# HaoZhongkai/DPOT

Measured on AMD Instinct MI355X. Metric: PDE samples/sec (128^2 x10 -> 1 rollout step), DPOT-Tiny train step, higher is better.
Workload: dtype f32

## Files before the change

dpot_amd/_lib.py:

```python
from __future__ import annotations

import ctypes as C
import os
import threading

HERE = os.path.dirname(os.path.abspath(__file__))
LIB_PATH = os.environ.get("DPOT_HIP_LIB") or os.path.join(HERE, "lib", "libdpot_hip.so")

c_fp = C.c_void_p
c_i = C.c_int
c_i64 = C.c_int64
c_f = C.c_float
c_d = C.c_double


class GemmDesc(C.Structure):
    _fields_ = [
        ("A", c_fp), ("B", c_fp), ("C", c_fp),
        ("M", C.c_int32), ("N", C.c_int32), ("K", C.c_int32),
        ("batch", C.c_int32),
        ("transA", C.c_int32), ("transB", C.c_int32),
        ("lda", C.c_int32), ("ldb", C.c_int32), ("ldc", C.c_int32),
        ("strideA", c_i64), ("strideB", c_i64), ("strideC", c_i64),
        ("bias", c_fp), ("strideBias", c_i64),
        ("act", C.c_int32), ("epi_mode", C.c_int32),
        ("aux", c_fp), ("ldaux", C.c_int32), ("strideAux", c_i64),
        ("preact", c_fp), ("ldpre", C.c_int32), ("stridePre", c_i64),
        ("res", c_fp), ("ldres", C.c_int32), ("res_div", C.c_int32), ("res_mod", C.c_int32),
        ("strideRes", c_i64),
        ("accumulate", C.c_int32), ("splitk", C.c_int32),
        ("workspace", c_fp),
        ("tile", C.c_int32),
        ("tag", C.c_int32),
        ("colsum_out", c_fp), ("strideColsum", c_i64), ("colsum_of", C.c_int32),
        ("precision", C.c_int32),
    ]


class PackJob(C.Structure):
    _fields_ = [("src", c_fp), ("dst", c_fp), ("rows", C.c_int32), ("K", C.c_int32), ("ld", C.c_int32),
                ("trans", C.c_int32)]


class AdamPackJob(C.Structure):
    _fields_ = [("off", C.c_int64), ("dst_rows", c_fp), ("dst_trans", c_fp), ("R", C.c_int32), ("K", C.c_int32),
                ("tile0", C.c_int32), ("pad_", C.c_int32)]


class AdamRange(C.Structure):
    _fields_ = [("start", C.c_int64), ("len", C.c_int64)]


class LambChunk(C.Structure):
    _fields_ = [("off", C.c_int64), ("len", C.c_int32), ("tensor", C.c_int32)]


class LambTensor(C.Structure):
    _fields_ = [("first_chunk", C.c_int32), ("n_chunks", C.c_int32)]


class LayoutJob(C.Structure):
    _fields_ = [("src", c_fp), ("add", c_fp), ("dst", c_fp), ("d0", C.c_int32), ("d1", C.c_int32), ("d2", C.c_int32),
                ("v0", C.c_int32), ("v1", C.c_int32), ("v2", C.c_int32), ("s0", C.c_int64), ("s1", C.c_int64),
                ("s2", C.c_int64)]


class AfnoPackJob(C.Structure):
    _fields_ = [("w", c_fp), ("b", c_fp), ("wbig", c_fp), ("bbig", c_fp), ("fwd", c_fp), ("bwd", c_fp)]


class SampleDesc(C.Structure):
    _fields_ = [("data", c_fp), ("H", C.c_int32), ("W", C.c_int32), ("T", C.c_int32), ("C", C.c_int32),
                ("t0", C.c_int32), ("reserved", C.c_int32)]


SIGNATURES = {
    "dpot_version": (c_i, []),
    "dpot_tune": (c_i, [C.c_char_p, c_i]),
    "dpot_last_error": (C.c_char_p, []),
    "dpot_gemm_f32": (c_i, [C.POINTER(GemmDesc), c_fp]),
    "dpot_gemm_workspace_bytes": (c_i64, [C.POINTER(GemmDesc)]),
    "dpot_gemm_auto_splitk": (c_i, [c_i, c_i, c_i, c_i]),
    "dpot_gemm_auto_splitk2": (c_i, [c_i, c_i, c_i, c_i, c_i]),
    "dpot_rfft2": (c_i, [c_fp, c_fp] + [c_i] * 8 + [c_fp]),
    "dpot_rfft2_norm_supported": (c_i, [c_i, c_i, c_i]),
    "dpot_rfft2_norm": (c_i, [c_fp] * 5 + [c_i, c_fp] + [c_i] * 8 + [c_fp]),
    "dpot_irfft2_norm": (c_i, [c_fp] * 6 + [c_i, c_fp] + [c_i] * 8 + [c_fp]),
    "dpot_irfft2": (c_i, [c_fp, c_fp, c_fp] + [c_i] * 8 + [c_fp]),
    "dpot_afno_pack": (c_i, [c_fp] * 4 + [c_i, c_i, c_fp]),
    "dpot_afno_pack_multi": (c_i, [C.POINTER(C.c_void_p)] * 4 + [c_i, c_i, c_i, c_fp]),
    "dpot_afno_unpack_grad": (c_i, [c_fp] * 4 + [c_i, c_i, c_fp]),
    "dpot_afno_mlp2_supported": (c_i, [c_i, c_i]),
    "dpot_afno_mlp2": (c_i, [c_fp] * 9 + [c_i] * 8 + [c_fp]),
    "dpot_afno_mlp3_supported": (c_i, [c_i, c_i]),
    "dpot_afno_mlp6_supported": (c_i, [c_i, c_i]),
    "dpot_afno_pack6_elems": (c_i64, [c_i, c_i]),
    "dpot_afno_pack6": (c_i, [c_fp] * 3 + [c_i] * 3 + [c_fp]),
    "dpot_afno_mlp6": (c_i, [c_fp] * 9 + [c_i] * 7 + [c_fp]),
    "dpot_afno_block_weights": (c_i, [c_fp] * 3 + [c_i, c_i, c_fp]),
    "dpot_afno_pack_all": (c_i, [c_fp, c_i, c_i, c_i, c_i, c_fp]),
    "dpot_groupnorm_ws_elems": (c_i64, [c_i] * 4),
    "dpot_groupnorm_fwd": (c_i, [c_fp] * 7 + [c_i] * 4 + [c_f, c_fp]),
    "dpot_groupnorm_bwd": (c_i, [c_fp] * 11 + [c_i] * 4 + [c_fp]),
    "dpot_groupnorm_bwd_packs_supported": (c_i, [c_i] * 3),
    "dpot_groupnorm_bwd_packs_rows": (c_i, [c_i] * 4),
    "dpot_groupnorm_bwd_packs": (c_i, [c_fp] * 12 + [c_i] * 4 + [c_fp]),
    "dpot_groupnorm_param_grads": (c_i, [C.c_void_p] * 3 + [c_i] * 3 + [c_fp]),
    "dpot_afno_fused_supported": (c_i, [c_i] * 7),
    "dpot_afno_fused_fwd": (c_i, [c_fp] * 19 + [c_i] * 9 + [c_f, c_fp]),
    "dpot_gn_dft_supported": (c_i, [c_i] * 4),
    "dpot_gn_rfft2": (c_i, [c_fp] * 6 + [c_i] * 8 + [c_f, c_fp]),
    "dpot_irfft2_gn": (c_i, [c_fp] * 12 + [c_i] * 9 + [c_f, c_fp]),
    "dpot_gn_bwd_rfft2": (c_i, [c_fp] * 8 + [c_i] * 9 + [c_fp]),
    "dpot_irfft2_gn_bwd": (c_i, [c_fp] * 9 + [c_i] * 9 + [c_fp]),
    "dpot_patchify": (c_i, [c_fp] * 5 + [c_i] * 6 + [c_fp]),
    "dpot_unpatchify": (c_i, [c_fp] * 2 + [c_i] * 6 + [c_fp]),
    "dpot_pixel_shuffle": (c_i, [c_fp] * 2 + [c_i] * 6 + [c_fp]),
    "dpot_copy2d_pad": (c_i, [c_fp, c_i, c_i, c_fp, c_i, c_i, c_fp]),
    "dpot_transpose2d": (c_i, [c_fp, c_fp, c_i, c_i, c_i, c_fp]),
    "dpot_colsum_parts": (c_i, [c_i]),
    "dpot_colsum": (c_i, [c_fp, c_i, c_i, c_i, c_fp, c_fp, c_fp]),
    "dpot_colsum_scatter": (c_i, [c_fp, c_i, c_i, c_i, c_fp, c_i, C.POINTER(C.c_int), C.POINTER(C.c_int),
                                  C.POINTER(C.c_void_p), c_fp]),
    "dpot_group_rowsum": (c_i, [c_fp, c_fp] + [c_i] * 4 + [c_fp]),
    "dpot_small_linear_supported": (c_i, [c_i] * 3),
    "dpot_small_linear": (c_i, [c_fp, c_i, c_fp, c_i, c_fp, c_fp, c_fp] + [c_i] * 5 + [c_fp]),
    "dpot_token_mean": (c_i, [c_fp, c_fp] + [c_i] * 3 + [c_fp]),
    "dpot_token_mean_bwd": (c_i, [c_fp] * 3 + [c_i] * 3 + [c_fp]),
    "dpot_bias_add": (c_i, [c_fp] * 3 + [c_i, c_i, c_fp]),
    "dpot_scale_shift": (c_i, [c_fp] * 4 + [c_i] * 3 + [c_fp]),
    "dpot_scale_shift_bwd": (c_i, [c_fp] * 6 + [c_i] * 3 + [c_fp]),
    "dpot_timeagg_scale_w": (c_i, [c_fp] * 4 + [c_i, c_i, c_fp]),
    "dpot_timeagg_scale_w_bwd": (c_i, [c_fp] * 6 + [c_i, c_i, c_fp]),
    "dpot_out_tail_partial_rows": (c_i, [c_i] * 4),
    "dpot_out_tail_partial_cols": (c_i, []),
    "dpot_out_tail_fwd": (c_i, [c_fp] * 6 + [c_i] * 6 + [c_fp]),
    "dpot_out_tail_bwd": (c_i, [c_fp] * 7 + [c_i] * 6 + [c_fp]),
    "dpot_rel_l2_chunks": (c_i, [c_i, c_i]),
    "dpot_rel_l2_fwd": (c_i, [c_fp] * 5 + [c_i] * 4 + [c_fp]),
    "dpot_rel_l2_bwd": (c_i, [c_fp] * 6 + [c_i] * 4 + [c_fp]),
    "dpot_sumsq": (c_i, [c_fp, c_i64, c_fp, c_fp, c_i, c_fp]),
    "dpot_adam_step": (c_i, [c_fp] * 4 + [c_i64, c_fp, c_fp, c_f, c_fp]),
    "dpot_adam_stage": (c_i, [c_fp, c_fp, c_f, c_d, c_d, c_f, c_f, c_f, c_i, c_fp]),
    "dpot_lamb_chunk_elems": (c_i, []),
    "dpot_lamb_step": (c_i, [c_fp] * 5 + [c_fp, c_f, c_fp, c_i, c_fp, c_i, c_fp, c_fp, c_i, c_fp]),
    "dpot_lamb_stage": (c_i, [c_fp, c_fp, c_d, c_d, c_d, c_f, c_f, c_f, c_f, c_i, c_i, c_fp]),
    "dpot_cls_ce_fwd": (c_i, [c_fp] * 4 + [c_i, c_i, c_fp]),
    "dpot_cls_ce_bwd": (c_i, [c_fp] * 5 + [c_i, c_i, c_fp]),
    "dpot_rel_l2_combine": (c_i, [c_fp, c_fp, c_i64, c_i, c_i, c_i, c_fp, c_fp]),
    "dpot_metrics_accum": (c_i, [c_fp] * 4 + [c_i, c_fp, c_f, c_i64, c_i64, c_i64, c_fp]),
    "dpot_noise_chunks": (c_i, [c_i, c_i]),
    "dpot_noise_inject": (c_i, [c_fp] * 4 + [c_f] + [c_i] * 3 + [c_fp]),
    "dpot_noise_inject_rng": (c_i, [c_fp] * 4 + [c_f] + [c_i] * 3 + [c_fp]),
    "dpot_noise_inject_bwd": (c_i, [c_fp] * 7 + [c_f] + [c_i] * 3 + [c_fp]),
    "dpot_window_slide": (c_i, [c_fp] * 3 + [c_i64] + [c_i] * 3 + [c_fp]),
    "dpot_window_slide_bwd": (c_i, [c_fp] * 3 + [c_i64] + [c_i] * 3 + [c_fp]),
    "dpot_resize_pad_window": (c_i, [c_fp, c_i, c_fp, c_fp] + [c_i] * 6 + [c_fp]),
    "dpot_spectral_resize_pad": (c_i, [c_i, c_i]),
    "dpot_spectral_resize": (c_i, [c_fp] * 7 + [c_i] * 6 + [c_fp]),
    "dpot_eval_metrics_pad": (c_i, [c_i, c_i]),
    "dpot_eval_metrics_max_size": (c_i, [c_i]),
    "dpot_eval_metrics_acc_elems": (c_i64, [c_i] * 4),
    "dpot_eval_metrics_stats": (c_i, [c_fp] * 9 + [c_i] * 4 + [c_fp]),
    "dpot_eval_metrics_finalize": (c_i, [c_fp] * 3 + [c_i] * 5 + [c_fp]),
    "dpot_panel_pack_weights": (c_i, [c_fp, c_i, c_i, c_fp]),
    "dpot_layout_jobs": (c_i, [c_fp, c_i, c_i64, c_fp]),
    "dpot_bf16_packed_elems": (c_i64, [c_i, c_i, c_i]),
    "dpot_bf16_pack_rows": (c_i, [c_fp, c_i, c_i, c_i, c_i, c_i, c_fp, c_fp]),
    "dpot_bf16_pack_jobs": (c_i, [c_fp, c_i, c_i, c_i, c_fp]),
    "dpot_adam_pack_supported": (c_i, [c_i, c_i]),
    "dpot_adam_step_packs": (c_i, [c_fp] * 6 + [c_f, c_fp, c_fp, c_i, c_fp, c_i, c_i, c_fp]),
    "dpot_gemm_bf16p_supported": (c_i, [c_i, c_i, c_i]),
    "dpot_gemm_bf16p": (c_i, [c_fp, c_fp, c_fp, c_fp, c_i, c_fp, c_i, c_fp, c_i, c_fp, c_i] + [c_i] * 7 + [c_fp] * 7),
    "dpot_gemm_bf16p_splitk": (c_i, [c_i, c_i, c_i]),
    "dpot_gemm_bf16p_pair_wanted": (c_i, [c_i] * 5),
    "dpot_gemm_bf16p_pair_splitk": (c_i, [c_i] * 5),
    "dpot_gemm_bf16p_kernel_kind": (c_i, [c_i] * 6),
    "dpot_gemm_bf16p_pair": (c_i, [c_fp, c_fp, c_fp, c_i, c_i, c_i, c_fp, c_fp, c_fp, c_i, c_i, c_i, c_i, c_i, c_fp, c_fp]),
    "dpot_gemm_tn_splitk": (c_i, [c_i] * 4),
    "dpot_mlp_wgrad2_splitk": (c_i, [c_i] * 3),
    "dpot_mlp_wgrad2_ws_elems": (c_i64, [c_i] * 3),
    "dpot_mlp_wgrad2": (c_i, [c_fp] * 4 + [c_i] * 3 + [c_fp] * 5 + [c_i, c_fp]),
    "dpot_afno_wgrad2_splitk": (c_i, [c_i] * 3),
    "dpot_afno_wgrad2_ws_elems": (c_i64, [c_i] * 3),
    "dpot_afno_wgrad2": (c_i, [c_fp] * 4 + [c_i] * 4 + [c_fp] * 5 + [c_i, c_fp]),
    "dpot_block_finalize": (c_i, [c_fp, c_i, c_i, c_i] + [c_fp] * 4 + [c_fp, c_i, c_i, c_i] + [c_fp] * 4 + [c_fp] * 3
                            + [c_i, c_i, c_i] + [c_fp] * 4 + [c_i, c_fp]),
    "dpot_bf16_pack_both_supported": (c_i, [c_i, c_i]),
    "dpot_bf16_pack_both": (c_i, [c_fp, c_i, c_i, c_i, c_fp, c_fp, c_fp, c_fp]),
    "dpot_bf16_pack_both_norm": (c_i, [c_fp, c_i, c_i, c_i, c_fp, c_fp, c_fp, c_fp, c_i, c_i, c_fp, c_fp, c_fp]),
    "dpot_embed_supported": (c_i, [c_i] * 5),
    "dpot_embed_wfrag_elems": (c_i, []),
    "dpot_embed_pack_w0": (c_i, [c_fp, c_i, c_fp, c_fp]),
    "dpot_embed_fwd": (c_i, [c_fp] * 5 + [c_i] * 6 + [c_fp]),
    "dpot_embed_wgrad_ws_elems": (c_i, [c_i] * 3),
    "dpot_embed_wgrad": (c_i, [c_fp] * 4 + [c_i] * 7 + [c_fp]),
    "dpot_gemm_panel_supported": (c_i, [c_i, c_i, c_i]),
    "dpot_gemm_panel": (c_i, [c_fp, c_i, c_fp, c_fp, c_fp, c_i, c_fp, c_i, c_fp, c_i, c_fp, c_i] + [c_i] * 5 + [c_fp]),
}

_lib = None
_lock = threading.Lock()


class DpotHipError(RuntimeError):
    pass


def lib_path() -> str:
    return LIB_PATH


def load():
    global _lib
    if _lib is not None:
        return _lib
    with _lock:
        if _lib is not None:
            return _lib
        if not os.path.exists(LIB_PATH):
            raise DpotHipError(
                f"{LIB_PATH} is missing - build it first (python -m dpot_amd.build, or __graft_entry__.build()). "
                "dpot_amd has no CPU / eager fallback by design.")
        lib = C.CDLL(LIB_PATH)
        for name, (res, args) in SIGNATURES.items():
            fn = getattr(lib, name)
            fn.restype = res
            fn.argtypes = args
        _lib = lib
    return _lib


def check(rc: int, what: str = "") -> None:
    if rc != 0:
# ... 3 lines not shown
```

dpot_amd/build.py:

```python
from __future__ import annotations

import os
import shutil
import subprocess
import sys
from concurrent.futures import ThreadPoolExecutor

HERE = os.path.dirname(os.path.abspath(__file__))
CSRC = os.path.join(HERE, "csrc")
LIBDIR = os.path.join(HERE, "lib")
LIB = os.path.join(LIBDIR, "libdpot_hip.so")
SOURCES = ["core.hip", "gemm.hip", "gemm_panel.hip", "gemm_tn.hip", "gemm_bf16p.hip", "afno_mlp.hip", "afno_mlp6.hip", "afno_fused.hip", "dft.hip", "norm.hip", "gn_dft.hip", "misc.hip", "loss_opt.hip", "metrics.hip", "tail.hip", "data.hip", "embed.hip", "resize.hip", "evalmetrics.hip"]
FLAGS = ["--offload-arch=gfx950", "-O3", "-std=c++17", "-fPIC", "-Wall", "-Wno-unused-function",
         "-Wno-pass-failed"]
EXTRA_FLAGS = {"afno_mlp6.hip": ["-fno-slp-vectorize"]}


def _hipcc() -> str:
    for cand in (os.environ.get("HIPCC"), shutil.which("hipcc"), "/opt/rocm/bin/hipcc"):
        if cand and os.path.exists(cand):
            return cand
    raise RuntimeError("hipcc not found (need ROCm >= 7.0 to build the gfx950 kernels)")


def _stale(target: str, deps) -> bool:
    if not os.path.exists(target):
        return True
    t = os.path.getmtime(target)
    return any(os.path.getmtime(d) > t for d in deps)


def build(force: bool = False, verbose: bool = True) -> str:
    hipcc = _hipcc()
    os.makedirs(LIBDIR, exist_ok=True)
    hdrs = [os.path.join(CSRC, "common.h"), os.path.join(CSRC, "dft_fast.h"), os.path.join(CSRC, "gemm_split.h"), os.path.join(CSRC, "gemm_epi.h"), os.path.join(CSRC, "gemm_bf16p_common.h"), os.path.join(os.path.dirname(HERE), "include", "dpot_hip.h")]
    objs, jobs = [], []
    for src in SOURCES:
        s = os.path.join(CSRC, src)
        o = os.path.join(LIBDIR, src.replace(".hip", ".o"))
        objs.append(o)
        if force or _stale(o, [s] + hdrs):
            jobs.append([hipcc] + FLAGS + EXTRA_FLAGS.get(src, []) + ["-c", s, "-o", o])

    def run(cmd):
        if verbose:
            print("[dpot_amd.build]", " ".join(cmd), flush=True)
        r = subprocess.run(cmd, capture_output=True, text=True)
        if r.returncode != 0:
            raise RuntimeError(f"hipcc failed:\n{' '.join(cmd)}\n{r.stdout}\n{r.stderr}")
        return r

    if jobs:
        with ThreadPoolExecutor(max_workers=min(6, len(jobs))) as ex:
            list(ex.map(run, jobs))
    if jobs or force or _stale(LIB, objs):
        run([hipcc, "--offload-arch=gfx950", "-shared", "-fPIC", "-o", LIB] + objs)
    return LIB


if __name__ == "__main__":
    print(build(force="--force" in sys.argv))
```

dpot_amd/csrc/gemm.hip:

```cpp
#include "common.h"
#include "gemm_epi.h"

namespace dpot {

constexpr int BK = 32;
constexpr int KPAD = 4;

template <int R, bool VEC>
__device__ __forceinline__ void load_kcontig(float4 (&reg)[R / 32], const float* __restrict__ base, int ld,
                                             int r0, int rmax, int k0, int kmax, int tid) {
#pragma unroll
  for (int i = 0; i < R / 32; ++i) {
    const int f = tid + 256 * i;
    const int r = r0 + (f >> 3);
    const int k = k0 + ((f & 7) << 2);
    const float* row = base + (long long)min(r, rmax - 1) * ld;
    float4 v;
    if constexpr (VEC) {
      v = *reinterpret_cast<const float4*>(row + min(k, kmax - 4));
    } else {
      const int kl = kmax - 1;
      v.x = row[min(k + 0, kl)]; v.y = row[min(k + 1, kl)]; v.z = row[min(k + 2, kl)]; v.w = row[min(k + 3, kl)];
    }
    reg[i] = v;
  }
}
template <int R, bool VEC>
__device__ __forceinline__ void load_rcontig(float4 (&reg)[R / 32], const float* __restrict__ base, int ld,
                                             int r0, int rmax, int k0, int kmax, int tid) {
  constexpr int F4_PER_ROW = R / 4;
#pragma unroll
  for (int i = 0; i < R / 32; ++i) {
    const int f = tid + 256 * i;
    const int k = k0 + f / F4_PER_ROW;
    const int r = r0 + ((f % F4_PER_ROW) << 2);
    const float* row = base + (long long)min(k, kmax - 1) * ld;
    float4 v;
    if constexpr (VEC) {
      v = *reinterpret_cast<const float4*>(row + min(r, rmax - 4));
    } else {
      const int rl = rmax - 1;
      v.x = row[min(r + 0, rl)]; v.y = row[min(r + 1, rl)]; v.z = row[min(r + 2, rl)]; v.w = row[min(r + 3, rl)];
    }
    reg[i] = v;
  }
}
template <int R>
__device__ __forceinline__ void zero_tail_kcontig(float* lds, int krem, int tid) {
  for (int idx = tid; idx < R * BK; idx += 256) {
    const int r = idx / BK, k = idx % BK;
    if (k >= krem) lds[r * (BK + KPAD) + k] = 0.f;
  }
}
template <int R>
__device__ __forceinline__ void zero_tail_rcontig(float* lds, int krem, int tid) {
  for (int idx = tid + krem * R; idx < BK * R; idx += 256) lds[idx] = 0.f;
}
template <int R>
__device__ __forceinline__ void store_kcontig(float* lds, const float4 (&reg)[R / 32], int tid) {
#pragma unroll
  for (int i = 0; i < R / 32; ++i) {
    const int f = tid + 256 * i;
    *reinterpret_cast<float4*>(&lds[(f >> 3) * (BK + KPAD) + ((f & 7) << 2)]) = reg[i];
  }
}
template <int R>
__device__ __forceinline__ void store_rcontig(float* lds, const float4 (&reg)[R / 32], int tid) {
  constexpr int F4_PER_ROW = R / 4;
#pragma unroll
  for (int i = 0; i < R / 32; ++i) {
    const int f = tid + 256 * i;
    *reinterpret_cast<float4*>(&lds[(f / F4_PER_ROW) * R + ((f % F4_PER_ROW) << 2)]) = reg[i];
  }
}

template <int R, bool KCONTIG>
struct TileLds {
  static constexpr int floats = KCONTIG ? R * (BK + KPAD) : BK * R;
};

template <int R, bool KCONTIG>
__device__ __forceinline__ float4 frag(const float* lds, int row, int kk, int kh) {
  if constexpr (KCONTIG) {
    return *reinterpret_cast<const float4*>(&lds[row * (BK + KPAD) + kk + 4 * kh]);
  } else {
    const float* p = &lds[(kk + 4 * kh) * R + row];
    return make_float4(p[0], p[R], p[2 * R], p[3 * R]);
  }
}

template <int BM, int BN, bool TA, bool TB, bool VEC, int TAG>
__global__ __launch_bounds__(256) void gemm_f32_kernel(const GemmArgs p) {
  constexpr bool A_KC = !TA;
  constexpr bool B_KC = TB;
  constexpr int TM = BM / 64, TN = BN / 64;
  constexpr int WM = BM / 2, WN = BN / 2;
  constexpr int OPER_FLOATS = TileLds<BM, A_KC>::floats + TileLds<BN, B_KC>::floats;
  constexpr int STAGE_FLOATS = 4 * 32 * EPI_LD;
  __shared__ __attribute__((aligned(16))) float smem[OPER_FLOATS > STAGE_FLOATS ? OPER_FLOATS : STAGE_FLOATS];
  float* As = smem;
  float* Bs = smem + TileLds<BM, A_KC>::floats;

  const int tid = threadIdx.x;
  const int lane = tid & 63, wave = tid >> 6;
  const int wm = wave >> 1, wn = wave & 1;
  const int li = lane & 31, kh = lane >> 5;

  const int ntiles = p.tilesM * p.tilesN;
  int tile;
  {
    const int bid = blockIdx.x;
    const int xcd = bid & 7, slot = bid >> 3;
    const int q = ntiles >> 3, r = ntiles & 7;
    tile = (xcd < r ? xcd * (q + 1) : r * (q + 1) + (xcd - r) * q) + slot;
  }
  const int tm_idx = tile / p.tilesN, tn_idx = tile % p.tilesN;
  const int m0 = tm_idx * BM, n0 = tn_idx * BN;
  const int zb = blockIdx.z / p.splits, zs = blockIdx.z % p.splits;
  const bool cs_on = (p.cs_of == 1 && tn_idx == 0) || (p.cs_of == 2 && tm_idx == 0);
  float cs_acc = 0.f;

  const float* A = p.A + zb * p.sA;
  const float* B = p.B + zb * p.sB;
  const int kbeg = zs * p.ktiles_per_split * BK;
  int kend = kbeg + p.ktiles_per_split * BK;
  if (kend > p.K) kend = p.K;
  const int nk = (kend > kbeg) ? (kend - kbeg + BK - 1) / BK : 0;

  f32x16 acc[TM][TN];
#pragma unroll
  for (int i = 0; i < TM; ++i)
#pragma unroll
    for (int j = 0; j < TN; ++j)
#pragma unroll
      for (int r = 0; r < 16; ++r) acc[i][j][r] = 0.f;

  float4 ra[BM / 32], rb[BN / 32];
  auto gload = [&](int k0) {
    if constexpr (A_KC) load_kcontig<BM, VEC>(ra, A, p.lda, m0, p.M, k0, kend, tid);
    else load_rcontig<BM, VEC>(ra, A, p.lda, m0, p.M, k0, kend, tid);
    if constexpr (B_KC) load_kcontig<BN, VEC>(rb, B, p.ldb, n0, p.N, k0, kend, tid);
    else load_rcontig<BN, VEC>(rb, B, p.ldb, n0, p.N, k0, kend, tid);
  };
  auto sstore = [&](int k0) {
    if constexpr (A_KC) store_kcontig<BM>(As, ra, tid); else store_rcontig<BM>(As, ra, tid);
    if constexpr (B_KC) store_kcontig<BN>(Bs, rb, tid); else store_rcontig<BN>(Bs, rb, tid);
    if (k0 + BK > kend) {
      __syncthreads();
      const int krem = kend - k0;
      if constexpr (A_KC) zero_tail_kcontig<BM>(As, krem, tid); else zero_tail_rcontig<BM>(As, krem, tid);
      if constexpr (B_KC) zero_tail_kcontig<BN>(Bs, krem, tid); else zero_tail_rcontig<BN>(Bs, krem, tid);
    }
  };

  if (nk > 0) {
    gload(kbeg);
    sstore(kbeg);
    __syncthreads();
    for (int kt = 0; kt < nk; ++kt) {
      if (kt + 1 < nk) gload(kbeg + (kt + 1) * BK);
      if (cs_on) {
        if constexpr (TA) {
          if (p.cs_of == 1)
            for (int k = tid / BM; k < BK; k += 256 / BM) cs_acc += As[k * BM + tid % BM];
        }
        if constexpr (!TB) {
          if (p.cs_of == 2)
            for (int k = tid / BN; k < BK; k += 256 / BN) cs_acc += Bs[k * BN + tid % BN];
        }
      }
#pragma unroll
      for (int kk = 0; kk < BK; kk += 8) {
        float4 af[TM], bf[TN];
#pragma unroll
        for (int i = 0; i < TM; ++i) af[i] = frag<BM, A_KC>(As, wm * WM + i * 32 + li, kk, kh);
#pragma unroll
        for (int j = 0; j < TN; ++j) bf[j] = frag<BN, B_KC>(Bs, wn * WN + j * 32 + li, kk, kh);
#pragma unroll
        for (int i = 0; i < TM; ++i)
#pragma unroll
          for (int j = 0; j < TN; ++j) {
            acc[i][j] = __builtin_amdgcn_mfma_f32_32x32x2f32(af[i].x, bf[j].x, acc[i][j], 0, 0, 0);
            acc[i][j] = __builtin_amdgcn_mfma_f32_32x32x2f32(af[i].y, bf[j].y, acc[i][j], 0, 0, 0);
            acc[i][j] = __builtin_amdgcn_mfma_f32_32x32x2f32(af[i].z, bf[j].z, acc[i][j], 0, 0, 0);
            acc[i][j] = __builtin_amdgcn_mfma_f32_32x32x2f32(af[i].w, bf[j].w, acc[i][j], 0, 0, 0);
          }
      }
      __syncthreads();
      if (kt + 1 < nk) {
        sstore(kbeg + (kt + 1) * BK);
        __syncthreads();
      }
    }
  }

  __syncthreads();
  if (cs_on) {
    const int R = p.cs_of == 1 ? BM : BN;
    smem[tid] = cs_acc;
    __syncthreads();
    if (tid < R) {
      float s = 0.f;
      for (int l = 0; l < 256 / R; ++l) s += smem[l * R + tid];
      const int L = p.cs_of == 1 ? p.M : p.N;
      const int g = (p.cs_of == 1 ? m0 : n0) + tid;
      if (g < L) {
        if (p.splits > 1)
          p.ws[(long long)p.splits * p.batch * p.M * p.N + ((long long)zs * p.batch + zb) * L + g] = s;
        else
          p.cs_out[zb * p.sCs + g] = s;
      }
    }
    __syncthreads();
  }
  float* stage = smem + wave * (32 * EPI_LD);
#define DPOT_EPI_FRAG(I, J)                                                                    \
  do {                                                                                         \
    const int n0f = n0 + wn * WN + (J) * 32;                                                   \
    const int m0f = m0 + wm * WM + (I) * 32;                                                   \
    if (p.splits > 1) {                                                                        \
      float* ws = p.ws + ((long long)zs * p.batch + zb) * p.M * p.N;                           \
      const int n = n0f + li;                                                                  \
      _Pragma("unroll") for (int r = 0; r < 16; ++r) {                                         \
        const int m = m0f + 4 * kh + (r & 3) + 8 * (r >> 2);                                   \
        if (m < p.M && n < p.N) ws[(long long)m * p.N + n] = acc[I][J][r];                     \
      }                                                                                        \
    } else {                                                                                   \
      epi_fragment(p.e, p.evec, zb, m0f, n0f, acc[I][J], stage, lane);                         \
    }                                                                                          \
  } while (0)
  DPOT_EPI_FRAG(0, 0);
  if constexpr (TN > 1) DPOT_EPI_FRAG(0, 1);
  if constexpr (TM > 1) {
    DPOT_EPI_FRAG(1, 0);
    if constexpr (TN > 1) DPOT_EPI_FRAG(1, 1);
  }
#undef DPOT_EPI_FRAG
}

__global__ __launch_bounds__(256) void splitk_reduce_kernel(const float* __restrict__ ws, int splits, int batch,
                                                            const EpiArgs e, float* __restrict__ cs_out,
                                                            long long sCs, int csL) {
// ... 237 lines not shown
```

dpot_amd/csrc/misc.hip:

```cpp
#include "common.h"

namespace dpot {

__global__ __launch_bounds__(256) void patchify_kernel(const float* __restrict__ x, const float* __restrict__ gx,
                                                       const float* __restrict__ gy, const float* __restrict__ gt,
                                                       float* __restrict__ A, int X, int Y, int T, int C, int P) {
  extern __shared__ float sm[];
  const int w = Y / P, h = X / P;
  const int site = blockIdx.x;
  const int py = site % w, px = (site / w) % h, b = site / (w * h);
  const int TC = T * C, run = P * TC, rp = run + 1;
  for (int i = 0; i < P; ++i) {
    const float* src = x + (((long long)b * X + px * P + i) * Y + py * P) * TC;
    for (int r = threadIdx.x; r < run; r += 256) sm[i * rp + r] = src[r];
  }
  __syncthreads();
  const int PP = P * P, K0 = (C + 3) * PP;
  float* out = A + (long long)site * T * K0;
  for (int k = threadIdx.x; k < K0; k += 256) {
    const int c = k / PP, rem = k - c * PP;
    const int i = rem / P, j = rem - i * P;
    if (c < C) {
      const float* s0 = sm + i * rp + j * TC + c;
      for (int t = 0; t < T; ++t) out[(long long)t * K0 + k] = s0[t * C];
// ... 51 lines not shown
                                  int dC) {
  const long long total = (long long)dR * dC;
  for (long long idx = blockIdx.x * 256ll + threadIdx.x; idx < total; idx += (long long)gridDim.x * 256) {
    const int r = (int)(idx / dC), c = (int)(idx % dC);
    dst[idx] = (r < sR && c < sC) ? src[(long long)r * sC + c] : 0.f;
  }
}

__global__ __launch_bounds__(256) void layout_jobs_kernel(const dpot_layout_job* __restrict__ jobs) {
  const dpot_layout_job j = jobs[blockIdx.y];
  const unsigned total = (unsigned)j.d0 * (unsigned)j.d1 * (unsigned)j.d2;
  const unsigned d12 = (unsigned)j.d1 * (unsigned)j.d2;
  for (unsigned idx = blockIdx.x * 256u + threadIdx.x; idx < total; idx += gridDim.x * 256u) {
    const unsigned i0 = idx / d12, r = idx - i0 * d12;
    const unsigned i1 = r / (unsigned)j.d2, i2 = r - i1 * (unsigned)j.d2;
    float v = 0.f;
    if ((int)i0 < j.v0 && (int)i1 < j.v1 && (int)i2 < j.v2) v = j.src[(long long)i0 * j.s0 + (long long)i1 * j.s1 + (long long)i2 * j.s2];
    if (j.add) v += j.add[i2];
    j.dst[idx] = v;
  }
}

__global__ __launch_bounds__(256) void transpose2d_kernel(const float* __restrict__ src, float* __restrict__ dst, int R,
                                                          int C) {
  __shared__ float tile[32][33];
  const long long boff = (long long)blockIdx.z * R * C;
  const int c0 = blockIdx.x * 32, r0 = blockIdx.y * 32;
  const int tx = threadIdx.x & 31, ty = threadIdx.x >> 5;
  for (int k = ty; k < 32; k += 8) {
    const int r = r0 + k, c = c0 + tx;
    if (r < R && c < C) tile[k][tx] = src[boff + (long long)r * C + c];
  }
  __syncthreads();
  for (int k = ty; k < 32; k += 8) {
    const int c = c0 + k, r = r0 + tx;
    if (r < R && c < C) dst[boff + (long long)c * R + r] = tile[tx][k];
  }
}

template <int CW>
__global__ __launch_bounds__(256) void colsum_kernel(const float* __restrict__ X, int M, int N, int ld,
                                                     float* __restrict__ out, int rows_per_part) {
  constexpr int RL = 256 / CW;
  __shared__ float red[RL][CW];
  const int tc = threadIdx.x % CW, tr = threadIdx.x / CW;
  const int n = blockIdx.x * CW + tc;
  const int m0 = blockIdx.y * rows_per_part;
  int m1 = m0 + rows_per_part;
  if (m1 > M) m1 = M;
  float s0 = 0.f, s1 = 0.f, s2 = 0.f, s3 = 0.f;
  if (n < N) {
    const float* p = X + n;
    int m = m0 + tr;
    for (; m + 3 * RL < m1; m += 4 * RL) {
      s0 += p[(long long)m * ld];
      s1 += p[(long long)(m + RL) * ld];
      s2 += p[(long long)(m + 2 * RL) * ld];
      s3 += p[(long long)(m + 3 * RL) * ld];
    }
    for (; m < m1; m += RL) s0 += p[(long long)m * ld];
  }
  red[tr][tc] = (s0 + s1) + (s2 + s3);
  __syncthreads();
  if (tr == 0 && n < N) {
    float s = 0.f;
#pragma unroll
    for (int r = 0; r < RL; ++r) s += red[r][tc];
    out[(long long)blockIdx.y * N + n] = s;
  }
}

__global__ __launch_bounds__(256) void group_rowsum_kernel(const float* __restrict__ X, float* __restrict__ out, int B,
                                                           int R, int T, int N) {
  __shared__ float red[4][64];
  const int tc = threadIdx.x & 63, tr = threadIdx.x >> 6;
  const int n = blockIdx.x * 64 + tc;
  const int r = blockIdx.y;
  float s0 = 0.f, s1 = 0.f;
  if (n < N) {
    const int BT = B * T;
    int q = tr;
    for (; q + 4 < BT; q += 8) {
      const int b0 = q / T, t0 = q % T, b1 = (q + 4) / T, t1 = (q + 4) % T;
      s0 += X[(((long long)b0 * R + r) * T + t0) * N + n];
      s1 += X[(((long long)b1 * R + r) * T + t1) * N + n];
    }
    for (; q < BT; q += 4) s0 += X[(((long long)(q / T) * R + r) * T + (q % T)) * N + n];
  }
  red[tr][tc] = s0 + s1;
  __syncthreads();
  if (tr == 0 && n < N) out[(long long)r * N + n] = (red[0][tc] + red[1][tc]) + (red[2][tc] + red[3][tc]);
}

__global__ __launch_bounds__(256) void token_mean_kernel(const float* __restrict__ x, float* __restrict__ y, int T,
                                                         int E) {
  __shared__ float red[4][64];
  const int tc = threadIdx.x & 63, tr = threadIdx.x >> 6;
  const int e = blockIdx.x * 64 + tc;
  const int b = blockIdx.y;
  float s0 = 0.f, s1 = 0.f;
  if (e < E) {
    const float* p = x + (long long)b * T * E + e;
    int t = tr;
    for (; t + 28 < T; t += 32) {
      const float a0 = p[(long long)t * E], a1 = p[(long long)(t + 4) * E], a2 = p[(long long)(t + 8) * E];
      const float a3 = p[(long long)(t + 12) * E], a4 = p[(long long)(t + 16) * E], a5 = p[(long long)(t + 20) * E];
      const float a6 = p[(long long)(t + 24) * E], a7 = p[(long long)(t + 28) * E];
      s0 += (a0 + a1) + (a2 + a3);
      s1 += (a4 + a5) + (a6 + a7);
    }
    for (; t < T; t += 4) s0 += p[(long long)t * E];
  }
  red[tr][tc] = s0 + s1;
  __syncthreads();
  if (tr == 0 && e < E)
    y[(long long)b * E + e] = ((red[0][tc] + red[1][tc]) + (red[2][tc] + red[3][tc])) / (float)T;
}
__global__ void token_mean_bwd_kernel(const float* __restrict__ dy, const float* __restrict__ add,
                                      float* __restrict__ dx, int T, int E, long long total) {
  const float inv = 1.0f / (float)T;
  for (long long idx = blockIdx.x * 256ll + threadIdx.x; idx < total; idx += (long long)gridDim.x * 256) {
    const int e = (int)(idx % E);
    const long long b = idx / ((long long)T * E);
    float v = dy[b * E + e] * inv;
    if (add) v += add[idx];
    dx[idx] = v;
  }
}

__global__ void bias_add_kernel(const float* __restrict__ x, const float* __restrict__ v, float* __restrict__ y, int N,
                                long long total) {
  for (long long i = blockIdx.x * 256ll + threadIdx.x; i < total; i += (long long)gridDim.x * 256)
    y[i] = (x ? x[i] : 0.f) + v[i % N];
}

__global__ void scale_shift_kernel(const float* __restrict__ x, const float* __restrict__ scale,
                                   const float* __restrict__ shift, float* __restrict__ y, int T, int E,
                                   long long total) {
  for (long long idx = blockIdx.x * 256ll + threadIdx.x; idx < total; idx += (long long)gridDim.x * 256) {
    const int e = (int)(idx % E);
    const long long b = idx / ((long long)T * E);
    y[idx] = fmaf(x[idx], scale[b * E + e], shift[b * E + e]);
  }
}

__global__ __launch_bounds__(256) void timeagg_scale_w_kernel(const float* __restrict__ w, const float* __restrict__ gamma,
                                                              const float* __restrict__ tt, float* __restrict__ ws,
                                                              int E) {
  const int i = blockIdx.x, t = blockIdx.y;
  const float cs = cosf(tt[t] * gamma[i]);
  const long long off = ((long long)t * E + i) * E;
  for (int j = threadIdx.x; j < E; j += 256) ws[off + j] = w[off + j] * cs;
}
__global__ __launch_bounds__(256) void timeagg_scale_w_bwd_kernel(const float* __restrict__ dws, const float* __restrict__ w,
                                                                  const float* __restrict__ gamma,
                                                                  const float* __restrict__ tt, float* __restrict__ dw,
                                                                  float* __restrict__ dgamma, int T, int E) {
  __shared__ float sh[16];
  const int i = blockIdx.x;
  const float ga = gamma[i];
  float acc = 0.f;
  for (int t = 0; t < T; ++t) {
    const float tv = tt[t];
    const float arg = tv * ga;
    const float cs = cosf(arg), coef = -sinf(arg) * tv;
    const long long off = ((long long)t * E + i) * E;
    float s = 0.f;
    for (int j = threadIdx.x; j < E; j += 256) {
      const float d = dws[off + j];
      dw[off + j] = d * cs;
      s = fmaf(d, w[off + j], s);
    }
    acc = fmaf(s, coef, acc);
  }
  const float dg = block_sum(acc, sh);
  if (dgamma && threadIdx.x == 0) dgamma[i] = dg;
}

__global__ __launch_bounds__(256) void scale_shift_bwd_kernel(const float* __restrict__ dy, const float* __restrict__ x,
                                                              const float* __restrict__ scale, float* __restrict__ dx,
                                                              float* __restrict__ dscale, float* __restrict__ dshift,
                                                              int T, int E) {
  __shared__ float s1[256], s2[256];
  const int b = blockIdx.y, e = blockIdx.x * 64 + (threadIdx.x & 63), tl = threadIdx.x >> 6;
  float a1 = 0.f, a2 = 0.f;
  if (e < E) {
    const float sc = scale[(long long)b * E + e];
    for (int t = tl; t < T; t += 4) {
      const long long idx = ((long long)b * T + t) * E + e;
      const float g = dy[idx];
      dx[idx] = g * sc;
      a1 = fmaf(g, x[idx], a1);
      a2 += g;
    }
  }
  s1[threadIdx.x] = a1;
  s2[threadIdx.x] = a2;
  __syncthreads();
  if (tl == 0 && e < E) {
    const int c = threadIdx.x;
    dscale[(long long)b * E + e] = (s1[c] + s1[c + 64]) + (s1[c + 128] + s1[c + 192]);
    dshift[(long long)b * E + e] = (s2[c] + s2[c + 64]) + (s2[c + 128] + s2[c + 192]);
  }
}

static inline unsigned grid_for(long long n, int cap = 8192) {
  long long g = (n + 255) / 256;
  if (g > cap) g = cap;
  if (g < 1) g = 1;
  return (unsigned)g;
}

}

using namespace dpot;

extern "C" int dpot_patchify(const float* x, const float* gx, const float* gy, const float* gt, float* A, int B,
                             int X, int Y, int T, int C, int P, dpot_stream_t stream) {
  DPOT_REQUIRE(x && gx && gy && gt && A, "patchify: null pointer");
  DPOT_REQUIRE(B > 0 && P > 0 && X % P == 0 && Y % P == 0 && T > 0 && C > 0, "patchify: bad shape");
  const size_t lds = sizeof(float) * (size_t)P * ((size_t)P * T * C + 1);
  DPOT_REQUIRE(lds <= 64 * 1024, "patchify: patch slab of %zu bytes exceeds 64 KiB", lds);
  const long long sites = (long long)B * (X / P) * (Y / P);
  DPOT_REQUIRE(sites < (1ll << 31), "patchify: too many sites");
  hipLaunchKernelGGL(patchify_kernel, dim3((unsigned)sites), dim3(256), lds, as_stream(stream), x, gx, gy, gt, A, X, Y,
                     T, C, P);
  return check_launch("patchify_kernel");
}

extern "C" int dpot_unpatchify(const float* dA, float* dx, int B, int X, int Y, int T, int C, int P,
                               dpot_stream_t stream) {
  DPOT_REQUIRE(dA && dx, "unpatchify: null pointer");
  DPOT_REQUIRE(B > 0 && P > 0 && X % P == 0 && Y % P == 0 && T > 0 && C > 0, "unpatchify: bad shape");
  const size_t lds = sizeof(float) * (size_t)P * ((size_t)P * T * C + 1);
  DPOT_REQUIRE(lds <= 64 * 1024, "unpatchify: patch slab of %zu bytes exceeds 64 KiB", lds);
  const long long sites = (long long)B * (X / P) * (Y / P);
  hipLaunchKernelGGL(unpatchify_kernel, dim3((unsigned)sites), dim3(256), lds, as_stream(stream), dA, dx, X, Y, T, C,
                     P);
  return check_launch("unpatchify_kernel");
}

extern "C" int dpot_pixel_shuffle(const float* z, float* out, int B, int h, int w, int P, int Cc, int inverse,
                                  dpot_stream_t stream) {
  DPOT_REQUIRE(z && out && B > 0 && h > 0 && w > 0 && P > 0 && Cc > 0, "pixel_shuffle: bad argument");
  const long long total = (long long)B * h * P * w * P * Cc;
  hipLaunchKernelGGL(pixel_shuffle_kernel, dim3(grid_for(total)), dim3(256), 0, as_stream(stream), z, out, h, w, P, Cc,
                     inverse, total);
  return check_launch("pixel_shuffle_kernel");
}

extern "C" int dpot_copy2d_pad(const float* src, int sR, int sC, float* dst, int dR, int dC, dpot_stream_t stream) {
  DPOT_REQUIRE(src && dst && sR > 0 && sC > 0 && dR > 0 && dC > 0, "copy2d_pad: bad argument");
  hipLaunchKernelGGL(copy2d_pad_kernel, dim3(grid_for((long long)dR * dC)), dim3(256), 0, as_stream(stream), src, sR,
                     sC, dst, dR, dC);
  return check_launch("copy2d_pad_kernel");
}

extern "C" int dpot_layout_jobs(const dpot_layout_job* jobs_dev, int njobs, int64_t max_elems, dpot_stream_t stream) {
  DPOT_REQUIRE(jobs_dev && njobs > 0 && njobs <= 65535 && max_elems > 0 && max_elems < (1ll << 31), "layout_jobs: bad argument");
  long long g = (max_elems + 255) / 256;
  if (g > 256) g = 256;
  hipLaunchKernelGGL(layout_jobs_kernel, dim3((unsigned)g, njobs), dim3(256), 0, as_stream(stream), jobs_dev);
  return check_launch("layout_jobs_kernel");
}

extern "C" int dpot_transpose2d(const float* src, float* dst, int nbatch, int R, int C, dpot_stream_t stream) {
  DPOT_REQUIRE(src && dst && nbatch > 0 && R > 0 && C > 0 && nbatch <= 65535 && cdiv(R, 32) <= 65535,
               "transpose2d: bad argument");
  hipLaunchKernelGGL(transpose2d_kernel, dim3(cdiv(C, 32), cdiv(R, 32), nbatch), dim3(256), 0, as_stream(stream), src,
                     dst, R, C);
  return check_launch("transpose2d_kernel");
}

extern "C" int dpot_colsum_parts(int M) {
  int parts = cdiv(M, 256);
  if (parts > 1024) parts = 1024;
  if (parts < 1) parts = 1;
  return parts;
}

static void launch_colsum(const float* X, int M, int N, int ld, float* out, int parts, hipStream_t s) {
  const int rpp = cdiv(M, parts);
  if (N <= 16) {
    hipLaunchKernelGGL(colsum_kernel<16>, dim3(cdiv(N, 16), parts), dim3(256), 0, s, X, M, N, ld, out, rpp);
  } else if (N <= 32) {
    hipLaunchKernelGGL(colsum_kernel<32>, dim3(cdiv(N, 32), parts), dim3(256), 0, s, X, M, N, ld, out, rpp);
  } else {
    hipLaunchKernelGGL(colsum_kernel<64>, dim3(cdiv(N, 64), parts), dim3(256), 0, s, X, M, N, ld, out, rpp);
  }
}

extern "C" int dpot_colsum(const float* X, int M, int N, int ld, float* out, float* part, dpot_stream_t stream) {
  DPOT_REQUIRE(X && out && part && M > 0 && N > 0 && ld >= N, "colsum: bad argument");
  int parts = dpot_colsum_parts(M);
  const int colblocks = cdiv(N, N <= 16 ? 16 : N <= 32 ? 32 : 64);
  const int want = cdiv(1024, colblocks);
  if (parts > want) parts = want;
  if (parts <= 1) {
    launch_colsum(X, M, N, ld, out, 1, as_stream(stream));
    return check_launch("colsum_kernel");
  }
  launch_colsum(X, M, N, ld, part, parts, as_stream(stream));
  int rc = check_launch("colsum_kernel");
  if (rc) return rc;
  launch_colsum(part, parts, N, N, out, 1, as_stream(stream));
  return check_launch("colsum_kernel(stage 2)");
// ... 4 lines not shown
  int start[8], len[8];
  float* dst[8];
};
__global__ __launch_bounds__(256) void colsum_scatter_kernel(const float* __restrict__ part, int parts, int N,
                                                             const ScatterSegs segs) {
  const int j = blockIdx.x * 256 + threadIdx.x;
  if (j >= N) return;
  float a = 0.f;
  for (int r = 0; r < parts; ++r) a += part[(long long)r * N + j];
  for (int s = 0; s < segs.n; ++s)
    if (j >= segs.start[s] && j < segs.start[s] + segs.len[s]) segs.dst[s][j - segs.start[s]] = a;
}

extern "C" int dpot_colsum_scatter(const float* X, int M, int N, int ld, float* part, int nseg, const int* seg_start,
                                   const int* seg_len, float* const* seg_dst, dpot_stream_t stream) {
  DPOT_REQUIRE(X && part && M > 0 && N > 0 && ld >= N && nseg > 0 && nseg <= 8 && seg_start && seg_len && seg_dst,
               "colsum_scatter: bad argument");
  ScatterSegs segs;
  segs.n = nseg;
  for (int s = 0; s < nseg; ++s) {
    DPOT_REQUIRE(seg_start[s] >= 0 && seg_len[s] > 0 && seg_start[s] + seg_len[s] <= N && seg_dst[s],
                 "colsum_scatter: bad segment %d", s);
    segs.start[s] = seg_start[s]; segs.len[s] = seg_len[s]; segs.dst[s] = seg_dst[s];
  }
  int parts = dpot_colsum_parts(M);
  const int want = cdiv(1024, cdiv(N, N <= 16 ? 16 : N <= 32 ? 32 : 64));
  if (parts > want) parts = want;
  if (parts < 1) parts = 1;
  launch_colsum(X, M, N, ld, part, parts, as_stream(stream));
  int rc = check_launch("colsum_kernel");
  if (rc) return rc;
  hipLaunchKernelGGL(colsum_scatter_kernel, dim3(cdiv(N, 256)), dim3(256), 0, as_stream(stream), (const float*)part,
                     parts, N, segs);
  return check_launch("colsum_scatter_kernel");
}

extern "C" int dpot_group_rowsum(const float* X, float* out, int B, int R, int T, int N, dpot_stream_t stream) {
  DPOT_REQUIRE(X && out && B > 0 && R > 0 && T > 0 && N > 0 && R <= 65535, "group_rowsum: bad argument");
  hipLaunchKernelGGL(group_rowsum_kernel, dim3(cdiv(N, 64), R), dim3(256), 0, as_stream(stream), X, out, B, R, T, N);
  return check_launch("group_rowsum_kernel");
}

namespace dpot {
constexpr int SL_ROWS = 32, SL_KCH = 512, SL_WAVES = 8;
template <int HALF>
__device__ __forceinline__ void sl_stage(float (&part)[SL_ROWS], int lane) {
  const bool hi = (lane & (2 * HALF)) != 0;
#pragma unroll
  for (int i = 0; i < HALF; ++i) {
    const float send = hi ? part[i] : part[HALF + i];
    const float keep = hi ? part[HALF + i] : part[i];
    part[i] = keep + __shfl_xor(send, 2 * HALF, 64);
  }
}
__global__ __launch_bounds__(64 * SL_WAVES) void small_linear_kernel(const float* __restrict__ x, int ldx,
                                                                     const float* __restrict__ W, int ldw,
                                                                     const float* __restrict__ bias,
                                                                     float* __restrict__ y, float* __restrict__ pre,
                                                                     int ldy, int M, int N, int K, int act) {
  extern __shared__ __attribute__((aligned(16))) float xs[];
  const int tid = threadIdx.x, lane = tid & 63, wave = tid >> 6;
  const int n_raw = blockIdx.x * SL_WAVES + wave;
  const int n = n_raw < N ? n_raw : N - 1;
  const float bn = bias ? bias[n] : 0.f;
  for (int m0 = 0; m0 < M; m0 += SL_ROWS) {
    float part[SL_ROWS];
#pragma unroll
    for (int i = 0; i < SL_ROWS; ++i) part[i] = 0.f;
    for (int k0 = 0; k0 < K; k0 += SL_KCH) {
      const float4 w0 = *reinterpret_cast<const float4*>(W + (long long)n * ldw + k0 + 4 * lane);
      const float4 w1 = *reinterpret_cast<const float4*>(W + (long long)n * ldw + k0 + 256 + 4 * lane);
      __syncthreads();
      float4 st[SL_ROWS * SL_KCH / 4 / (64 * SL_WAVES)];
#pragma unroll
      for (int j = 0; j < SL_ROWS * SL_KCH / 4 / (64 * SL_WAVES); ++j) {
        const int q = tid + j * 64 * SL_WAVES;
        const int m = m0 + (q >> 7) < M ? m0 + (q >> 7) : M - 1;
        st[j] = *reinterpret_cast<const float4*>(x + (long long)m * ldx + k0 + 4 * (q & 127));
      }
#pragma unroll
      for (int j = 0; j < SL_ROWS * SL_KCH / 4 / (64 * SL_WAVES); ++j)
        *reinterpret_cast<float4*>(xs + 4 * (tid + j * 64 * SL_WAVES)) = st[j];
      __syncthreads();
#pragma unroll
      for (int i = 0; i < SL_ROWS; ++i) {
        const float4 a = *reinterpret_cast<const float4*>(xs + i * SL_KCH + 4 * lane);
        const float4 b = *reinterpret_cast<const float4*>(xs + i * SL_KCH + 256 + 4 * lane);
        float t = part[i];
        t = fmaf(a.x, w0.x, t); t = fmaf(a.y, w0.y, t); t = fmaf(a.z, w0.z, t); t = fmaf(a.w, w0.w, t);
        t = fmaf(b.x, w1.x, t); t = fmaf(b.y, w1.y, t); t = fmaf(b.z, w1.z, t); t = fmaf(b.w, w1.w, t);
        part[i] = t;
      }
    }
    sl_stage<16>(part, lane); sl_stage<8>(part, lane); sl_stage<4>(part, lane); sl_stage<2>(part, lane);
    sl_stage<1>(part, lane);
    const float v = part[0] + __shfl_xor(part[0], 1, 64) + bn;
    const int m = m0 + (lane >> 1);
    if ((lane & 1) == 0 && m < M && n_raw < N) {
      if (pre) pre[(long long)m * ldy + n] = v;
      y[(long long)m * ldy + n] = act_fwd(act, v);
    }
  }
}

}

extern "C" int dpot_token_mean(const float* x, float* y, int B, int T, int E, dpot_stream_t stream) {
  DPOT_REQUIRE(x && y && B > 0 && T > 0 && E > 0 && B <= 65535, "token_mean: bad argument");
  hipLaunchKernelGGL(token_mean_kernel, dim3(cdiv(E, 64), B), dim3(256), 0, as_stream(stream), x, y, T, E);
  return check_launch("token_mean_kernel");
}

extern "C" int dpot_token_mean_bwd(const float* dy, const float* add, float* dx, int B, int T, int E,
                                   dpot_stream_t stream) {
  DPOT_REQUIRE(dy && dx && B > 0 && T > 0 && E > 0, "token_mean_bwd: bad argument");
  const long long total = (long long)B * T * E;
  hipLaunchKernelGGL(token_mean_bwd_kernel, dim3(grid_for(total)), dim3(256), 0, as_stream(stream), dy, add, dx, T, E,
                     total);
  return check_launch("token_mean_bwd_kernel");
}

extern "C" int dpot_bias_add(const float* x, const float* v, float* y, int R, int N, dpot_stream_t stream) {
  DPOT_REQUIRE(v && y && R > 0 && N > 0, "bias_add: bad argument");
  const long long total = (long long)R * N;
  hipLaunchKernelGGL(bias_add_kernel, dim3(grid_for(total)), dim3(256), 0, as_stream(stream), x, v, y, N, total);
  return check_launch("bias_add_kernel");
}

extern "C" int dpot_scale_shift(const float* x, const float* scale, const float* shift, float* y, int B, int T, int E,
                                dpot_stream_t stream) {
  DPOT_REQUIRE(x && scale && shift && y && B > 0 && T > 0 && E > 0, "scale_shift: bad argument");
  const long long total = (long long)B * T * E;
  hipLaunchKernelGGL(scale_shift_kernel, dim3(grid_for(total)), dim3(256), 0, as_stream(stream), x, scale, shift, y, T,
                     E, total);
  return check_launch("scale_shift_kernel");
}

extern "C" int dpot_scale_shift_bwd(const float* dy, const float* x, const float* scale, float* dx, float* dscale,
                                    float* dshift, int B, int T, int E, dpot_stream_t stream) {
  DPOT_REQUIRE(dy && x && scale && dx && dscale && dshift && B > 0 && B <= 65535 && T > 0 && E > 0,
               "scale_shift_bwd: bad argument");
  hipLaunchKernelGGL(scale_shift_bwd_kernel, dim3((unsigned)cdiv(E, 64), B), dim3(256), 0, as_stream(stream), dy, x,
                     scale, dx, dscale, dshift, T, E);
  return check_launch("scale_shift_bwd_kernel");
}

extern "C" int dpot_timeagg_scale_w(const float* w, const float* gamma, const float* tt, float* ws, int T, int E,
                                    dpot_stream_t stream) {
  DPOT_REQUIRE(w && gamma && tt && ws && T > 0 && E > 0 && T <= 65535, "timeagg_scale_w: bad argument");
  hipLaunchKernelGGL(timeagg_scale_w_kernel, dim3(E, T), dim3(256), 0, as_stream(stream), w, gamma, tt, ws, E);
  return check_launch("timeagg_scale_w_kernel");
}

extern "C" int dpot_timeagg_scale_w_bwd(const float* dws, const float* w, const float* gamma, const float* tt,
                                        float* dw, float* dgamma, int T, int E, dpot_stream_t stream) {
  DPOT_REQUIRE(dws && w && gamma && tt && dw && T > 0 && E > 0, "timeagg_scale_w_bwd: bad argument");
  hipLaunchKernelGGL(timeagg_scale_w_bwd_kernel, dim3(E), dim3(256), 0, as_stream(stream), dws, w, gamma, tt, dw,
                     dgamma, T, E);
  return check_launch("timeagg_scale_w_bwd_kernel");
}

extern "C" int dpot_small_linear_supported(int M, int N, int K) {
  return M > 0 && M <= 128 && N > 0 && K >= SL_KCH && K % SL_KCH == 0 ? 1 : 0;
}

extern "C" int dpot_small_linear(const float* x, int ldx, const float* W, int ldw, const float* bias, float* y, float* pre,
                                 int ldy, int M, int N, int K, int act, dpot_stream_t stream) {
  DPOT_REQUIRE(x && W && y, "small_linear: null operand");
  DPOT_REQUIRE(dpot_small_linear_supported(M, N, K), "small_linear: unsupported shape M=%d N=%d K=%d", M, N, K);
  DPOT_REQUIRE(ldx >= K && ldw >= K && ldy >= N && ldx % 4 == 0 && ldw % 4 == 0 && aligned16(x) && aligned16(W),
               "small_linear: bad leading dimension / alignment");
  const size_t lds = sizeof(float) * SL_ROWS * SL_KCH;
  static const hipError_t attr = hipFuncSetAttribute(reinterpret_cast<const void*>(small_linear_kernel),
                                                     hipFuncAttributeMaxDynamicSharedMemorySize, (int)lds);
  DPOT_REQUIRE(attr == hipSuccess, "small_linear: cannot reserve %zu bytes of LDS", lds);
  hipLaunchKernelGGL(small_linear_kernel, dim3((unsigned)cdiv(N, SL_WAVES)), dim3(64 * SL_WAVES), lds, as_stream(stream),
                     x, ldx, W, ldw, bias, y, pre, ldy, M, N, K, act);
  return check_launch("small_linear_kernel");
}
```

dpot_amd/functional.py:

```python
from __future__ import annotations

import os
from collections import OrderedDict
from typing import Optional

import torch

from . import ops
from .ops import EPI_ACT, EPI_DACT

Tensor = torch.Tensor


def _pad4(n: int) -> int:
    return (n + 3) // 4 * 4


class _Sink:
    __slots__ = ("fp", "i")

    def __init__(self, param: Optional[Tensor], needed: bool):
        s = getattr(param, "_dpot_grad_slot", None) if (needed and param is not None) else None
        self.fp, self.i = s if s is not None else (None, -1)
        if self.fp is not None:
            self.fp.pending[self.i] += 1

    def out(self) -> Optional[Tensor]:
        if self.fp is None or self.fp.filled[self.i]:
            return None
        return self.fp.grad_views[self.i]

    def done(self, t: Optional[Tensor]) -> Optional[Tensor]:
        if self.fp is None or t is None:
            return t
        fp, i = self.fp, self.i
        view = fp.grad_views[i]
        if t.data_ptr() != view.data_ptr():
            view.add_(t.reshape(view.shape))
        fp.filled[i] = True
        fp.pending[i] -= 1
        if fp.pending[i] == 0:
            fp.fire(i)
        return None

    def skip(self) -> None:
        if self.fp is None:
            return
        fp, i = self.fp, self.i
        fp.pending[i] -= 1
        if fp.pending[i] == 0 and fp.filled[i]:
            fp.fire(i)


def _epoch_of(sinks):
    for sk in sinks:
        if sk.fp is not None:
            return sk.fp, sk.fp.epoch
    return None


def _check_epoch(ctx, what: str) -> None:
    rec = ctx.weights_epoch
    if rec is not None and rec[0].epoch != rec[1]:
        raise RuntimeError(f"{what}.backward: the parameters were updated (optimiser step) after this forward ran; its "
                           "packed weights have been overwritten.  Run backward before the step, or re-run the forward.")


def _sinks(ctx, params, first_index: int):
    return [_Sink(p, ctx.needs_input_grad[first_index + k]) for k, p in enumerate(params)]


def embed_grid_matrix(gx, gy, gt, X: int, Y: int, T: int, Cc: int, P: int):
    z = torch.zeros(1, X, Y, T, Cc, dtype=torch.float32, device=gx.device)
    return ops.patchify(z, gx, gy, gt, P)[:, Cc * P * P:].contiguous()


def embed_layout_jobs(pos, w0, b0, w2, b2):
    hid, E = w0.shape[0], w2.shape[0]
    K0 = w0[0].numel()
    hidp = _pad4(hid)
    tok = pos.shape[2] * pos.shape[3]
    return [(w0, None, (1, hidp, K0), (1, hid, K0), (0, K0, 1)),
            (b0, None, (1, 1, hidp), (1, 1, hid), (0, 0, 1)),
            (w2, None, (1, E, hidp), (1, E, hid), (0, hid, 1)),
            (pos, b2, (1, tok, E), (1, tok, E), (0, 1, tok))]


def embed_derived(pos, w0, b0, w2, b2, taw, tagamma, tt, T: int, grid=None, layouts=None):
    hid, E = w0.shape[0], w2.shape[0]
    K0 = w0[0].numel()
    hidp = _pad4(hid)
    tok = pos.shape[2] * pos.shape[3]
    dev = pos.device
    if layouts is not None:
        w0p, b0p, w2p, posb = layouts[0].view(hidp, K0), layouts[1].view(hidp), layouts[2].view(E, hidp), layouts[3].view(tok, E)
    else:
        w0p = ops.copy2d_pad(w0, hid, K0, hidp, K0)
        b0p = ops.copy2d_pad(b0, 1, hid, 1, hidp).view(hidp)
        w2p = ops.copy2d_pad(w2, E, hid, E, hidp)
        posT = ops.transpose2d(pos, 1, E, tok).view(tok, E)
        posb = ops.bias_add(posT, b2)
    ws = ops.timeagg_scale_w(taw, tagamma, tt) if tagamma is not None else taw
    V = torch.empty(T * hidp, E, dtype=torch.float32, device=dev)
    ops.gemm(w2p, ws, V, hidp, E, E, transA=True, lda=hidp, ldb=E, ldc=E, batch=T, strideA=0, strideB=E * E,
             strideC=hidp * E)
    wsum = ops.colsum(ws, T, E * E).view(E, E)
    cc = torch.empty(tok, E, dtype=torch.float32, device=dev)
    ops.gemm(posb, wsum, cc, tok, E, E, lda=E, ldb=E, ldc=E)
    wfrag = bt = None
    if grid is not None:
        kg = grid.shape[1]
        wfrag = ops.embed_pack_w0(w0)
        bt = torch.empty(grid.shape[0], hidp, dtype=torch.float32, device=dev)
        ops.gemm(grid, w0p[:, K0 - kg:], bt, grid.shape[0], hidp, kg, transB=True, lda=kg, ldb=K0, ldc=hidp, bias=b0p)
    return w0p, b0p, w2p, posb, ws, V, wsum, cc, wfrag, bt, grid


class EmbedFn(torch.autograd.Function):

    @staticmethod
    def forward(ctx, x, pos, w0, b0, w2, b2, taw, tagamma, gx, gy, gt, tt, P: int, act: int, derived=None):
        ops.capture_precision(ctx)
        x = x.contiguous()
        B, X, Y, T, Cc = x.shape
        h, w = X // P, Y // P
        tok = h * w
        hid, E = w0.shape[0], w2.shape[0]
        K0 = (Cc + 3) * P * P
        hidp = _pad4(hid)
        dev = x.device
        M = B * tok

        implicit = derived is not None and derived[8] is not None
        A0 = None if implicit else ops.patchify(x, gx, gy, gt, P)
        if derived is None:
            derived = embed_derived(pos, w0, b0, w2, b2, taw, tagamma, tt, T)
        w0p, b0p, w2p, posb, ws, V, wsum, cc, wfrag, bt, grid = derived
        if implicit:
            Hh, Hpre = ops.embed_fwd(x, wfrag, bt, hidp, act)
        else:
            Hh, Hpre = ops.linear_fwd(A0, w0p, b0p, act=act, save_pre=True)
        Yl = torch.empty(M, E, dtype=torch.float32, device=dev)
        ops.gemm(Hh, V, Yl, M, E, T * hidp, lda=T * hidp, ldb=E, ldc=E, res=cc, ldres=E, res_mod=tok)
        ctx.implicit = implicit
        ctx.save_for_backward(x if implicit else A0, Hpre, Hh, w0p, w2p, ws, V, wsum, posb, taw, tagamma, tt,
                              grid if implicit else x.new_empty(0))
        ctx.dims = (B, X, Y, T, Cc, P, h, w, hid, hidp, E, K0, act)
        ctx.sinks = _sinks(ctx, (pos, w0, b0, w2, b2, taw, tagamma), 1)
        ctx.weights_epoch = _epoch_of(ctx.sinks)
        return Yl.view(B, tok, E)

    @staticmethod
    @ops.with_ctx_precision
    def backward(ctx, dY):
        _check_epoch(ctx, "EmbedFn")
        A0, Hpre, Hh, w0p, w2p, ws, V, wsum, posb, taw, tagamma, tt, grid = ctx.saved_tensors
        B, X, Y, T, Cc, P, h, w, hid, hidp, E, K0, act = ctx.dims
        s_pos, s_w0, s_b0, s_w2, s_b2, s_taw, s_gamma = ctx.sinks
        tok = h * w
        M, M0 = B * tok, B * tok * T
        dev = dY.device
        dY = dY.contiguous().view(M, E)
        dHpre = torch.empty(M0, hidp, dtype=torch.float32, device=dev)
        ops.gemm(dY, V, dHpre, M, T * hidp, E, transB=True, lda=E, ldb=E, ldc=T * hidp, act=act, mode=EPI_DACT,
                 aux=Hpre, ldaux=T * hidp)
        dV = torch.empty(T * hidp, E, dtype=torch.float32, device=dev)
        ops.gemm(Hh, dY, dV, T * hidp, E, M, transA=True, lda=T * hidp, ldb=E, ldc=E,
                 splitk=ops.auto_splitk(T * hidp, E, M, tn=True))
        dc = ops.group_rowsum(dY, B, tok, 1, E)
        dwsum = torch.empty(E, E, dtype=torch.float32, device=dev)
        ops.gemm(posb, dc, dwsum, E, E, tok, transA=True, lda=E, ldb=E, ldc=E, splitk=ops.auto_splitk(E, E, tok, tn=True))
        dposb = torch.empty(tok, E, dtype=torch.float32, device=dev)
        ops.gemm(dc, wsum, dposb, tok, E, E, transB=True, lda=E, ldb=E, ldc=E)
        dpos = s_pos.done(ops.transpose2d(dposb, 1, tok, E, out=s_pos.out()).view(1, E, h, w))
        db2 = s_b2.done(ops.colsum(dposb, tok, E, out=s_b2.out()))
        dw2_t = torch.empty(T, E, hidp, dtype=torch.float32, device=dev)
        ops.gemm(ws, dV, dw2_t, E, hidp, E, transB=True, lda=E, ldb=E, ldc=hidp, batch=T, strideA=E * E,
                 strideB=hidp * E, strideC=E * hidp)
        dw2p = ops.colsum(dw2_t, T, E * hidp).view(E, hidp)
        dw2 = s_w2.done(ops.copy2d_pad(dw2p, E, hidp, E, hid, out=s_w2.out()).view(E, hid, 1, 1))
        dws = s_taw.out() if tagamma is None else None
        dws = ops._out(dws, (T, E, E), dev)
        ops.gemm(w2p, dV, dws, E, E, hidp, lda=hidp, ldb=E, ldc=E, batch=T, strideA=0, strideB=hidp * E,
                 strideC=E * E, res=dwsum, ldres=E, strideRes=0)
        if tagamma is not None:
            dtaw, dgamma = ops.timeagg_scale_w_bwd(dws, taw, tagamma, tt, out_dw=s_taw.out(),
                                                   out_dgamma=s_gamma.out())
            dtaw, dgamma = s_taw.done(dtaw), s_gamma.done(dgamma)
        else:
            dtaw, dgamma = s_taw.done(dws), None
        if ctx.implicit:
            db0 = s_b0.done(ops.colsum(dHpre, M0, hid, ld=hidp, out=s_b0.out()))
            dw0 = ops._out(s_w0.out(), (hid, K0), dev)
            ops.embed_wgrad(A0, dHpre, dw0, hid)
            dHs = ops.group_rowsum(dHpre, B, tok * T, 1, hidp)
            kg = grid.shape[1]
            ops.gemm(dHs, grid, dw0[:, K0 - kg:], hid, kg, tok * T, transA=True, lda=hidp, ldb=kg, ldc=K0)
            dw0 = s_w0.done(dw0.view(hid, Cc + 3, P, P))
        elif hid == hidp:
            dw0p, db0 = ops.linear_bwd_wb(dHpre, A0, None, s_b0.out())
            db0 = s_b0.done(db0)
        else:
            db0 = s_b0.done(ops.colsum(dHpre, M0, hid, ld=hidp, out=s_b0.out()))
            dw0p = ops.linear_bwd_weight(dHpre, A0)
        if not ctx.implicit:
            dw0 = s_w0.done(ops.copy2d_pad(dw0p, hidp, K0, hid, K0, out=s_w0.out()).view(hid, Cc + 3, P, P))
        dx = None
        if ctx.needs_input_grad[0]:
            dA0 = ops.linear_bwd_data(dHpre, w0p)
            dx = ops.unpatchify(dA0, B, X, Y, T, Cc, P)
        return dx, dpos, dw0, db0, dw2, db2, dtaw, dgamma, None, None, None, None, None, None, None


X6_MIN_FLOP = 3.0e9


def mlp_pack_kind(E: int, mh: int, M: Optional[int] = None) -> Optional[str]:
    eff = ops.effective_mlp_precision()
    Mq = 128 if M is None else M
    bf_ok = ops.gemm_bf16p_supported(Mq, mh, E) and ops.gemm_bf16p_supported(Mq, E, mh)
    if bf_ok and eff == ops.GEMM_BF16:
        return "bf16"
    if eff == ops.GEMM_F32 and ops.panel_enabled() and ops.gemm_panel_supported(Mq, mh, E) \
            and ops.gemm_panel_supported(Mq, E, mh):
        return "f32"
    return None


def _mlp_panel_mode(mlp_pk, M, E, mh, mp) -> int:
    if mlp_pk is None:
        return 0
    kind = getattr(mlp_pk, "kind", "f32")
    if kind != mlp_pack_kind(E, mh, M):
        return 0
    if kind == "f32":
        return 1
    ok = ops.gemm_bf16p_supported(E, mh, M) and ops.gemm_bf16p_supported(mh, E, M)
    return 2 if ok else 0


def _p6_of(packed, which: int):
    a, b = getattr(packed[0], "p6", None), getattr(packed[1], "p6", None)
    if a is None or b is None or a[which] is None or b[which] is None or not ops.afno_mlp6_wanted():
        return None
    return a[which], b[which]


def _mixer_core(S, packed, dims, afno_layout=None):
    B, tok, E, h, w, nb, bs, mx, my, mh, act = dims
    Mm = B * mx * my
    dev = S.device
    (wb1, bb1, wb1T, _), (wb2, bb2, wb2T, _) = packed
    if wb1T is not None:
        lay = afno_layout if afno_layout is not None else getattr(packed[0], "layout", 0)
        p6 = _p6_of(packed, 0)
        if p6 is not None:
            wb1T, wb2T, lay = p6[0], p6[1], 2
        O2, O1pre, O1 = ops.afno_mlp2(S, wb1T, bb1, wb2T, bb2, nb, bs, act, mode=0, want_pre=True, want_mid=False,
                                      layout=lay)
    else:
        O1 = torch.empty(Mm, 2 * E, dtype=torch.float32, device=dev)
        O1pre = torch.empty_like(O1)
        kw = dict(lda=2 * E, ldb=2 * bs, ldc=2 * E, batch=nb, strideA=2 * bs, strideB=4 * bs * bs, strideC=2 * bs,
                  strideBias=2 * bs, tag=1)
        ops.gemm(S, wb1, O1, Mm, 2 * bs, 2 * bs, bias=bb1, act=act, mode=EPI_ACT, preact=O1pre, ldpre=2 * E,
                 stridePre=2 * bs, **kw)
        O2 = torch.empty_like(O1)
        ops.gemm(O1, wb2, O2, Mm, 2 * bs, 2 * bs, bias=bb2, **kw)
    return O2, O1pre, O1


def _mixer_fwd(xn1, packed, dims, afno_layout=None, norm=None):
    B, tok, E, h, w, nb, bs, mx, my, mh, act = dims
    lay = afno_layout if afno_layout is not None else getattr(packed[0], "layout", 0)
    if norm is None and packed[0][2] is not None and ops.afno_fused_supported(h, w, E, nb, mx, my, G=0, B=B, layout=lay):
        S, O1pre, y1 = ops.afno_fused_fwd(xn1, None, None, packed[0][2], packed[0][1], packed[1][2], packed[1][1], None,
                                          None, h, w, nb, mx, my, act)[:3]
        return y1, S, O1pre, None
    S = ops.rfft2(xn1, h, w, nb, mx, my, 0, norm=norm)
    O2, O1pre, O1 = _mixer_core(S, packed, dims, afno_layout)
    y1 = ops.irfft2(O2, B, h, w, E, nb, mx, my, 1, res=xn1, res_norm=norm)
    return y1, S, O1pre, O1


def _mixer_core_bwd(dO2, S, O1pre, O1, wb1, wb2, dims, fused, afno_layout, sinks, pending=None):
    B, tok, E, h, w, nb, bs, mx, my, mh, act = dims
    s_w1, s_b1, s_w2, s_b2 = sinks
    Mm = B * mx * my
    dev = dO2.device
    kw = dict(lda=2 * E, ldb=2 * bs, ldc=2 * E, batch=nb, strideA=2 * bs, strideB=4 * bs * bs, strideC=2 * bs)
    sk = max(2, ops.auto_splitk(2 * bs, 2 * bs, Mm, nb, tn=True))
    wkw = dict(transA=True, lda=2 * E, ldb=2 * E, ldc=2 * bs, batch=nb, strideA=2 * bs, strideB=2 * bs,
               strideC=4 * bs * bs, splitk=sk, mode=ops.EPI_AFNO_WGRAD)
    sk2 = ops.afno_wgrad2_splitk(Mm, nb, bs) if fused and S.stride(0) == 2 * E else 0
    if fused:
        dS, O1r, dO1pre = ops.afno_mlp2(dO2, wb2, None, wb1, None, nb, bs, act, mode=1, aux=O1pre, want_mid=True,
                                        want_pre=O1 is None, layout=afno_layout)
        if O1 is None:
            O1 = O1r
    if not sk2:
        dw2, db2 = ops._out(s_w2.out(), (2, nb, bs, bs), dev), ops._out(s_b2.out(), (2, nb, bs), dev)
        ops.gemm(O1, dO2, dw2, 2 * bs, 2 * bs, Mm, colsum_out=db2, colsum_of=2, **wkw)
        dw2, db2 = s_w2.done(dw2), s_b2.done(db2)
    if not fused:
        dO1pre = torch.empty(Mm, 2 * E, dtype=torch.float32, device=dev)
        ops.gemm(dO2, wb2, dO1pre, Mm, 2 * bs, 2 * bs, transB=True, act=act, mode=EPI_DACT, aux=O1pre,
                 ldaux=2 * E, strideAux=2 * bs, **kw)
    if sk2:
        dw1, db1 = ops._out(s_w1.out(), (2, nb, bs, bs), dev), ops._out(s_b1.out(), (2, nb, bs), dev)
        dw2, db2 = ops._out(s_w2.out(), (2, nb, bs, bs), dev), ops._out(s_b2.out(), (2, nb, bs), dev)
        if pending is not None:
            pending["afno"] = ops.afno_wgrad2(S, dO1pre, O1, dO2, nb, bs, dw1, db1, dw2, db2, sk2, defer=True)
        else:
            ops.afno_wgrad2(S, dO1pre, O1, dO2, nb, bs, dw1, db1, dw2, db2, sk2)
            dw1, db1, dw2, db2 = s_w1.done(dw1), s_b1.done(db1), s_w2.done(dw2), s_b2.done(db2)
    else:
        dw1, db1 = ops._out(s_w1.out(), (2, nb, bs, bs), dev), ops._out(s_b1.out(), (2, nb, bs), dev)
        ops.gemm(S, dO1pre, dw1, 2 * bs, 2 * bs, Mm, colsum_out=db1, colsum_of=2, **wkw)
        dw1, db1 = s_w1.done(dw1), s_b1.done(db1)
    if not fused:
        dS = torch.empty(Mm, 2 * E, dtype=torch.float32, device=dev)
        ops.gemm(dO1pre, wb1, dS, Mm, 2 * bs, 2 * bs, transB=True, **kw)
    return dS, dw1, db1, dw2, db2


def _mixer_bwd(dy1, S, O1pre, O1, wb1, wb2, dims, fused, afno_layout, sinks, pending=None):
    B, tok, E, h, w, nb, bs, mx, my, mh, act = dims
    dO2 = ops.rfft2(dy1, h, w, nb, mx, my, 1)
    dS, dw1, db1, dw2, db2 = _mixer_core_bwd(dO2, S, O1pre, O1, wb1, wb2, dims, fused, afno_layout, sinks, pending)
    dxn1 = ops.irfft2(dS, B, h, w, E, nb, mx, my, 0, res=dy1)
    return dxn1, dw1, db1, dw2, db2


class AFNO2DFn(torch.autograd.Function):

    @staticmethod
    def forward(ctx, x, w1, b1, w2, b2, h: int, w: int, nb: int, modes: int, act: int, packed=None):
        ops.capture_precision(ctx)
        x = x.contiguous()
        B, tok, E = x.shape
        bs = E // nb
        mx, my = min(modes, h), min(modes, w // 2 + 1)
        if packed is None:
            packed = tuple(ops.AfnoPacks([(w1, b1), (w2, b2)]).refresh())
        dims = (B, tok, E, h, w, nb, bs, mx, my, 0, act)
        y1, S, O1pre, O1 = _mixer_fwd(x, packed, dims)
        ctx.fused = packed[0][2] is not None
        wb1, wb2 = (packed[0][3], packed[1][3]) if ctx.fused else (packed[0][0], packed[1][0])
        ctx.afno_layout = getattr(packed[0], "layout", 0) if ctx.fused else 0
        ctx.p6b = _p6_of(packed, 1) if ctx.fused else None
        ctx.save_for_backward(S, O1pre, O1, wb1, wb2)
        ctx.dims = dims
        ctx.sinks = _sinks(ctx, (w1, b1, w2, b2), 1)
        ctx.weights_epoch = _epoch_of(ctx.sinks)
        return y1

    @staticmethod
    @ops.with_ctx_precision
    def backward(ctx, dy):
# ... 504 lines not shown
```

dpot_amd/ops.py:

```python
from __future__ import annotations

import ctypes as C
import contextlib
import functools
import threading
import os
from typing import Optional, Tuple

import torch

from . import _lib
from ._lib import GemmDesc, check

Tensor = torch.Tensor

ACT_IDS = {None: 0, "none": 0, "gelu": 1, "tanh": 2, "sigmoid": 3, "relu": 4, "leaky_relu": 5, "softplus": 6,
           "ELU": 7, "silu": 8}
EPI_LINEAR, EPI_ACT, EPI_DACT, EPI_AFNO_WGRAD = 0, 1, 2, 3
GEMM_F32, GEMM_BF16X6, GEMM_AUTO, GEMM_BF16 = 0, 1, 2, 3
_PRECISIONS = {"f32": GEMM_F32, "bf16x6": GEMM_BF16X6, "auto": GEMM_AUTO, "bf16": GEMM_BF16}
_gemm_precision = _PRECISIONS[os.environ.get("DPOT_GEMM_PRECISION", "f32")]


def set_gemm_precision(name: str) -> None:
    global _gemm_precision
    _gemm_precision = _PRECISIONS[name]


def gemm_precision() -> str:
    return {v: k for k, v in _PRECISIONS.items()}[_cur_gemm()]


_mlp_precision = _PRECISIONS[os.environ["DPOT_MLP_PRECISION"]] if os.environ.get("DPOT_MLP_PRECISION") else None


def set_mlp_precision(name: Optional[str]) -> None:
    global _mlp_precision
    _mlp_precision = None if name is None else _PRECISIONS[name]


_tls = threading.local()
_UNSET = object()


def _cur_gemm() -> int:
    v = getattr(_tls, "gemm", None)
    return _gemm_precision if v is None else v


def _cur_mlp() -> Optional[int]:
    v = getattr(_tls, "mlp", _UNSET)
    return _mlp_precision if v is _UNSET else v


def _code(prec) -> int:
    return _PRECISIONS[prec] if isinstance(prec, str) else int(prec)


@contextlib.contextmanager
def mlp_precision_scope(prec):
    if prec is None:
        yield
        return
    prev = getattr(_tls, "mlp", _UNSET)
    _tls.mlp = _code(prec)
    try:
        yield
    finally:
        if prev is _UNSET:
            del _tls.mlp
        else:
            _tls.mlp = prev


@contextlib.contextmanager
def gemm_precision_scope(prec):
    if prec is None:
        yield
        return
    prev = getattr(_tls, "gemm", None)
    _tls.gemm = _code(prec)
    try:
        yield
    finally:
        _tls.gemm = prev


@contextlib.contextmanager
def precision_scope(gemm=None, mlp=None):
    with gemm_precision_scope(gemm), mlp_precision_scope(mlp):
        yield


def with_ctx_precision(backward):
    @functools.wraps(backward)
    def wrapper(ctx, *grads):
        with precision_scope(getattr(ctx, "gemm_precision", None), getattr(ctx, "mlp_precision", None)):
            return backward(ctx, *grads)
    return wrapper


def capture_precision(ctx) -> None:
    ctx.gemm_precision = _cur_gemm()
    ctx.mlp_precision = effective_mlp_precision()


def effective_mlp_precision() -> int:
    m = _cur_mlp()
    return m if m is not None else _cur_gemm()


def mlp_precision() -> Optional[int]:
    return _cur_mlp()


TUNE_KEYS = {
    "mixer": (3, "AFNO mixer MLP: 3 = three-product fused kernel (afno_mlp3), 4 = four-product fused kernel (afno_mlp2), "
                 "0 = two generic GEMM launches"),
    "afno_layer": (-1, "one-launch AFNO layer forward (afno_fused_fwd): -1 = where it measured faster (>= 80 % full last "
                       "round of (sample, block) workgroups), 0 = never, 1 = wherever supported"),
    "gn_fuse": (1, "0 = GroupNorm as its own kernels: not fused with the mixer's DFTs, never applied on the load of its consumer"),
    "panel": (1, "0 = generic GEMM kernels instead of the pre-packed-weight panel GEMM, the token-contraction weight-gradient "
                 "kernels (gemm_tn) and their two-layer launches"),
    "wgrad_gauss": (1, "0 = four-product AFNO weight gradients instead of the three-product forms"),
    "bf16p_bd": (1, "0 = the LDS-DMA bf16 GEMM kernels of rounds 2-3 for every launch instead of the B-direct kernels"),
    "bf16p_shape": (1, "0 = none of the bf16 GEMM shape heuristics: 128 x 256 tiles only, column-major tile order, eight waves, "
                       "un-paired weight gradients"),
    "packs": (1, "0 = bf16 packs by separate pack passes only: none from the one-launch AFNO layer, the GroupNorm backward or Adam"),
    "pack_both": (1, "0 = bf16 channel MLP without the pack-both path (one pack pass per operand form, fp32 pre-activation saved)"),
    "fused_small": (1, "0 = separate small launches: per-block reduce launches, eight layout launches, torch ops for the cls head"),
    "embed_implicit": (1, "0 = explicit patch matrix + GEMM instead of the implicit-GEMM patch embedding"),
    "mixer6": (1, "bf16x6 mixer kernel afno_mlp6 under gemm_precision 'auto' / 'bf16x6': 1 = where it measured faster (96 channels "
                  "per block: DPOT-L), 2 = wherever supported (also 128), 0 = never (the fp32 matrix-core kernels)"),
}


_tune_parsed = ("", {})


def _parse_tune():
    global _tune_parsed
    env = os.environ.get("DPOT_TUNE", "")
    if env == _tune_parsed[0]:
        return _tune_parsed[1]
    out = {}
    for kv in env.split(","):
        kv = kv.strip()
        if not kv:
            continue
        k, _, v = kv.partition("=")
        if k not in TUNE_KEYS:
            raise ValueError(f"DPOT_TUNE: unknown key {k!r} (known: {', '.join(TUNE_KEYS)})")
        out[k] = int(v)
    _tune_parsed = (env, out)
    return out


def tune(key: str, default: Optional[int] = None) -> int:
    d = TUNE_KEYS[key][0] if default is None else default
    return _parse_tune().get(key, d)


def _stream() -> int:
    return torch.cuda.current_stream().cuda_stream


def _req(t: Tensor, name: str = "tensor") -> Tensor:
    if not t.is_cuda:
        raise _lib.DpotHipError(f"{name} must live on the MI355X (got a {t.device} tensor): dpot_amd has no CPU path")
    if t.dtype != torch.float32:
        raise _lib.DpotHipError(f"{name} must be float32, got {t.dtype}")
    if not t.is_contiguous():
        raise _lib.DpotHipError(f"{name} must be contiguous")
    return t


def _p(t: Optional[Tensor]) -> Optional[int]:
    return None if t is None else t.data_ptr()


def auto_splitk(M: int, N: int, K: int, batch: int = 1, precision: Optional[int] = None, tn: bool = False) -> int:
    lib = _lib.load()
    prec = _cur_gemm() if precision is None else precision
    if tn and prec == GEMM_F32:
        s = lib.dpot_gemm_tn_splitk(M, N, K, batch)
        if s > 0:
            return s
    return lib.dpot_gemm_auto_splitk2(M, N, K, batch, prec)


def gemm(A: Tensor, B: Tensor, C_: Tensor, M: int, N: int, K: int, *, transA: bool = False, transB: bool = False,
         lda: int, ldb: int, ldc: int, batch: int = 1, strideA: int = 0, strideB: int = 0, strideC: int = 0,
         bias: Optional[Tensor] = None, strideBias: int = 0, act: int = 0, mode: int = EPI_LINEAR,
         aux: Optional[Tensor] = None, ldaux: int = 0, strideAux: int = 0,
         preact: Optional[Tensor] = None, ldpre: int = 0, stridePre: int = 0,
         res: Optional[Tensor] = None, ldres: int = 0, res_div: int = 0, res_mod: int = 0, strideRes: int = 0,
         accumulate: bool = False, splitk: Optional[int] = None, tile: int = 0, tag: int = 0,
         colsum_out: Optional[Tensor] = None, colsum_of: int = 0, strideColsum: int = 0,
         precision: Optional[int] = None) -> Tensor:
    lib = _lib.load()
    d = GemmDesc()
    d.A, d.B, d.C = A.data_ptr(), B.data_ptr(), C_.data_ptr()
    d.M, d.N, d.K, d.batch = M, N, K, batch
    d.transA, d.transB = int(transA), int(transB)
    d.lda, d.ldb, d.ldc = lda, ldb, ldc
    d.strideA, d.strideB, d.strideC = strideA, strideB, strideC
    d.bias, d.strideBias = _p(bias), strideBias
    d.act, d.epi_mode = act, mode
    d.aux, d.ldaux, d.strideAux = _p(aux), ldaux, strideAux
    d.preact, d.ldpre, d.stridePre = _p(preact), ldpre, stridePre
    d.res, d.ldres, d.res_div, d.res_mod, d.strideRes = _p(res), ldres, res_div, res_mod, strideRes
    d.accumulate = int(accumulate)
    d.tile = tile
    d.tag = tag
    d.precision = _cur_gemm() if precision is None else precision
    if splitk is None:
        small = ((M + 63) // 64) * ((N + 63) // 64) * batch <= 128
        splitk = auto_splitk(M, N, K, batch, precision=d.precision) if small else 1
    d.colsum_out, d.colsum_of, d.strideColsum = _p(colsum_out), (colsum_of if colsum_out is not None else 0), strideColsum
    ws = None
    if splitk > 1:
        L = M if d.colsum_of == 1 else N if d.colsum_of == 2 else 0
        ws = torch.empty(splitk * batch * (M * N + L), dtype=torch.float32, device=A.device)
        d.splitk, d.workspace = splitk, ws.data_ptr()
    else:
        d.splitk, d.workspace = 1, None
    check(lib.dpot_gemm_f32(C.byref(d), _stream()), "gemm_f32")
    return C_


def panel_enabled() -> bool:
    return tune("panel") != 0 and _cur_gemm() == GEMM_F32


def gemm_panel_supported(M: int, N: int, K: int) -> bool:
    return bool(_lib.load().dpot_gemm_panel_supported(M, N, K))


def _device_table(struct, entries, dev) -> Tensor:
    import numpy as np
    arr = (struct * len(entries))(*(struct(*e) for e in entries))
    return torch.from_numpy(np.frombuffer(bytearray(arr), dtype=np.uint8)).to(dev)


class PanelPacks:

    def __init__(self, jobs, bf16: bool = False, planes: int = 1):
        dev = jobs[0][0].device
        self.bf16 = bf16
        self.planes = planes if bf16 else 0
        if bf16:
            lib = _lib.load()
            self.bufs = [torch.empty(lib.dpot_bf16_packed_elems(rows, K, planes), dtype=torch.bfloat16, device=dev)
                         for _, rows, K, _, _ in jobs]
        else:
            self.bufs = [torch.empty(rows * K, dtype=torch.float32, device=dev) for _, rows, K, _, _ in jobs]
        self.table = _device_table(_lib.PackJob, [(src.data_ptr(), dst.data_ptr(), rows, K, ld, int(trans))
                                                  for (src, rows, K, ld, trans), dst in zip(jobs, self.bufs)], dev)
        self.n = len(jobs)
        self.max_elems = max(rows * K for _, rows, K, _, _ in jobs)
        self.jobs = list(jobs)

    def refresh(self) -> None:
        lib = _lib.load()
        if self.bf16:
            check(lib.dpot_bf16_pack_jobs(self.table.data_ptr(), self.n, self.max_elems, self.planes, _stream()),
                  "bf16_pack_jobs")
        else:
            check(lib.dpot_panel_pack_weights(self.table.data_ptr(), self.n, self.max_elems, _stream()), "pack_weights")


class LayoutJobs:

    def __init__(self, jobs):
        dev = jobs[0][0].device
        self.out = [torch.empty(d, dtype=torch.float32, device=dev) for _, _, d, _, _ in jobs]
        self.sources = [(j[0], j[1]) for j in jobs]
        self.table = _device_table(_lib.LayoutJob, [(src.data_ptr(), _p(add), dst.data_ptr(), *d, *v, *st)
                                                    for (src, add, d, v, st), dst in zip(jobs, self.out)], dev)
        self.n = len(jobs)
        self.max_elems = max(d[0] * d[1] * d[2] for _, _, d, _, _ in jobs)

    def refresh(self):
        check(_lib.load().dpot_layout_jobs(self.table.data_ptr(), self.n, self.max_elems, _stream()), "layout_jobs")
        return self.out


def gemm_panel(A: Tensor, Wpacked: Tensor, N: int, *, bias: Optional[Tensor] = None, act: int = 0,
               mode: int = EPI_LINEAR, aux: Optional[Tensor] = None, res: Optional[Tensor] = None,
               save_pre: bool = False) -> Tuple[Tensor, Optional[Tensor]]:
    M, K = A.shape
    out = torch.empty(M, N, dtype=torch.float32, device=A.device)
    pre = torch.empty_like(out) if save_pre else None
    check(_lib.load().dpot_gemm_panel(A.data_ptr(), A.stride(0), Wpacked.data_ptr(), _p(bias), _p(aux),
                                      aux.stride(0) if aux is not None else 0, _p(res),
                                      res.stride(0) if res is not None else 0, _p(pre), N, out.data_ptr(), N, M, N, K,
                                      act, mode, _stream()), "gemm_panel")
    return out, pre


def gemm_bf16p_supported(M: int, N: int, K: int) -> bool:
    return bool(_lib.load().dpot_gemm_bf16p_supported(M, N, K))


class MlpPacks(tuple):

    def __new__(cls, bufs, kind: str):
        self = super().__new__(cls, bufs)
        self.kind = kind
        return self

    @property
    def planes(self) -> int:
        return {"f32": 0, "bf16": 1, "bf16x6": 3}[self.kind]


def bf16_pack_rows(x: Tensor, trans: bool = False, planes: int = 1) -> Tensor:
    lib = _lib.load()
    if trans:
        K, M = x.shape
    else:
        M, K = x.shape
    out = torch.empty(lib.dpot_bf16_packed_elems(M, K, planes), dtype=torch.bfloat16, device=x.device)
    check(lib.dpot_bf16_pack_rows(x.data_ptr(), x.stride(0), M, K, int(trans), planes, out.data_ptr(), _stream()),
          "bf16_pack_rows")
    return out


def bf16_pack_both_supported(rows: int, K: int) -> bool:
    return bool(_lib.load().dpot_bf16_pack_both_supported(rows, K))


def bf16_pack_both(x: Tensor, want_rows: bool = True, want_trans: bool = True, colsum_out: Optional[Tensor] = None,
                   want_colsum: bool = False, norm=None, defer_colsum: bool = False):
    lib = _lib.load()
    M, K = x.shape
    pr = torch.empty(lib.dpot_bf16_packed_elems(M, K, 1), dtype=torch.bfloat16, device=x.device) if want_rows else None
    pt = torch.empty(lib.dpot_bf16_packed_elems(K, M, 1), dtype=torch.bfloat16, device=x.device) if want_trans else None
    if norm is not None:
        mean, rstd, gamma, beta, rps = norm
        assert not want_colsum
        check(lib.dpot_bf16_pack_both_norm(x.data_ptr(), x.stride(0), M, K, mean.data_ptr(), rstd.data_ptr(),
                                           gamma.data_ptr(), beta.data_ptr(), rps, mean.shape[1], _p(pr), _p(pt), _stream()),
              "bf16_pack_both_norm")
        return pr, pt, None
    part = torch.empty(M // 64, K, dtype=torch.float32, device=x.device) if want_colsum else None
    check(lib.dpot_bf16_pack_both(x.data_ptr(), x.stride(0), M, K, _p(pr), _p(pt), _p(part), _stream()), "bf16_pack_both")
    if want_colsum and defer_colsum:
        return pr, pt, (part, M // 64, K, _out(colsum_out, (K,), x.device))
    cs = colsum(part, M // 64, K, out=colsum_out) if want_colsum else None
    return pr, pt, cs


def gemm_bf16p(Ap: Tensor, Wp: Tensor, M: int, N: int, K: int, *, bias: Optional[Tensor] = None, act: int = 0,
               mode: int = EPI_LINEAR, aux: Optional[Tensor] = None, res: Optional[Tensor] = None,
               save_pre: bool = False, out: Optional[Tensor] = None, splitk: Optional[int] = None,
               planes: int = 1) -> Tuple[Tensor, Optional[Tensor]]:
    C_, pre, _, _, _ = gemm_bf16p_packed(Ap, Wp, M, N, K, bias=bias, act=act, mode=mode, aux=aux, res=res,
                                         save_pre=save_pre, out=out, splitk=splitk, planes=planes)
    return C_, pre


def gemm_bf16p_pair_wanted(M0: int, N0: int, M1: int, N1: int, K: int) -> bool:
    return bool(_lib.load().dpot_gemm_bf16p_pair_wanted(M0, N0, M1, N1, K))


BF16P_KERNEL_KINDS = {0: "dpot::gemm_bf16p_kernel (8 compute + 4 loader waves, LDS-DMA)",
                      1: "dpot::gemm_bf16p_duo_kernel (two 8-wave workgroups per CU)",
                      2: "dpot::gemm_bf16p_bd_kernel<8,1,3> (B-direct: W fragments straight from global memory into registers, "
                         "only the A panel through LDS; eight 128 x 32 waves)",
                      3: "dpot::gemm_bf16p_bd_kernel<8,2,3> (B-direct: W fragments straight from global memory into registers, "
                         "only the A panel through LDS; four 128 x 64 waves, two workgroups per CU)",
                      4: "dpot::gemm_bf16x6p_kernel (fp32-accurate three-plane split)"}


def gemm_bf16p_kernel_name(M: int, N: int, K: int, splitk: int = 1, planes: int = 1, packed_outputs: bool = False) -> str:
    k = _lib.load().dpot_gemm_bf16p_kernel_kind(M, N, K, splitk, planes, int(packed_outputs))
    return BF16P_KERNEL_KINDS.get(k & 7, f"kind {k}") + (" on 128 x 192 tiles" if k >= 8 else "")


def gemm_bf16p_pair(A0: Tensor, W0: Tensor, M0: int, N0: int, A1: Tensor, W1: Tensor, M1: int, N1: int, K: int,
                    out0: Optional[Tensor] = None, out1: Optional[Tensor] = None,
                    splitk: Optional[int] = None) -> Tuple[Tensor, Tensor]:
# ... 497 lines not shown
                                        dx.data_ptr(), part.data_ptr(), spec.data_ptr(), B, h, w, E, G, nb, mx, my,
                                        col_weights, _stream()), "gn_bwd_rfft2")
    return dx, part, spec


def irfft2_gn_bwd(spec: Tensor, res: Tensor, xin: Tensor, mean: Tensor, rstd: Tensor, gamma: Tensor, h: int, w: int,
                  nb: int, mx: int, my: int, add: Optional[Tensor] = None, G: int = 8, col_weights: int = 0):
    B, _, E = xin.shape
    dx = torch.empty_like(xin)
    part = torch.empty(2, B, E, dtype=torch.float32, device=xin.device)
    check(_lib.load().dpot_irfft2_gn_bwd(spec.data_ptr(), res.data_ptr(), xin.data_ptr(), mean.data_ptr(), rstd.data_ptr(),
                                         gamma.data_ptr(), _p(add), dx.data_ptr(), part.data_ptr(), B, h, w, E, G, nb, mx,
                                         my, col_weights, _stream()), "irfft2_gn_bwd")
    return dx, part


def patchify(x: Tensor, gx: Tensor, gy: Tensor, gt: Tensor, P: int) -> Tensor:
    B, X, Y, T, Cc = x.shape
    K0 = (Cc + 3) * P * P
    A = torch.empty(B * (X // P) * (Y // P) * T, K0, dtype=torch.float32, device=x.device)
    check(_lib.load().dpot_patchify(x.data_ptr(), gx.data_ptr(), gy.data_ptr(), gt.data_ptr(), A.data_ptr(), B, X, Y,
                                    T, Cc, P, _stream()), "patchify")
    return A


def embed_supported(Cc: int, P: int, T: int, hid: int, w: int) -> bool:
    return (tune("embed_implicit") != 0
            and bool(_lib.load().dpot_embed_supported(Cc, P, T, hid, w)))


def embed_pack_w0(w0: Tensor) -> Tensor:
    lib = _lib.load()
    wf = torch.empty(lib.dpot_embed_wfrag_elems(), dtype=torch.float32, device=w0.device)
    check(lib.dpot_embed_pack_w0(w0.data_ptr(), w0.shape[0], wf.data_ptr(), _stream()), "embed_pack_w0")
    return wf


def embed_fwd(x: Tensor, wfrag: Tensor, btab: Tensor, hidp: int, act: int) -> Tuple[Tensor, Tensor]:
    B, X, Y, T, _ = x.shape
    M0 = B * (X // 8) * (Y // 8) * T
    hpre = torch.empty(M0, hidp, dtype=torch.float32, device=x.device)
    hh = torch.empty_like(hpre)
    check(_lib.load().dpot_embed_fwd(x.data_ptr(), wfrag.data_ptr(), btab.data_ptr(), hpre.data_ptr(), hh.data_ptr(),
                                     B, X, Y, T, hidp, act, _stream()), "embed_fwd")
    return hh, hpre


def embed_wgrad(x: Tensor, dhpre: Tensor, dw0: Tensor, hid: int) -> Tensor:
    lib = _lib.load()
    B, X, Y, T, _ = x.shape
    ws = torch.empty(lib.dpot_embed_wgrad_ws_elems(B, X, Y), dtype=torch.float32, device=x.device)
    check(lib.dpot_embed_wgrad(x.data_ptr(), dhpre.data_ptr(), ws.data_ptr(), dw0.data_ptr(), dw0.stride(0), hid, B, X,
                               Y, T, dhpre.shape[1], _stream()), "embed_wgrad")
    return dw0


def unpatchify(dA: Tensor, B: int, X: int, Y: int, T: int, Cc: int, P: int) -> Tensor:
    dx = torch.empty(B, X, Y, T, Cc, dtype=torch.float32, device=dA.device)
    check(_lib.load().dpot_unpatchify(dA.data_ptr(), dx.data_ptr(), B, X, Y, T, Cc, P, _stream()), "unpatchify")
    return dx


def pixel_shuffle(z: Tensor, B: int, h: int, w: int, P: int, Cc: int, inverse: bool = False) -> Tensor:
    out = torch.empty(B * h * w * P * P, Cc, dtype=torch.float32, device=z.device)
    if not inverse:
        out = out.view(B, h * P, w * P, Cc)
        check(_lib.load().dpot_pixel_shuffle(z.data_ptr(), out.data_ptr(), B, h, w, P, Cc, 0, _stream()),
              "pixel_shuffle")
    else:
        check(_lib.load().dpot_pixel_shuffle(z.data_ptr(), out.data_ptr(), B, h, w, P, Cc, 1, _stream()),
              "pixel_shuffle")
    return out


def copy2d_pad(src: Tensor, sR: int, sC: int, dR: int, dC: int, out: Optional[Tensor] = None) -> Tensor:
    dst = _out(out, (dR, dC), src.device)
    check(_lib.load().dpot_copy2d_pad(src.data_ptr(), sR, sC, dst.data_ptr(), dR, dC, _stream()), "copy2d_pad")
    return dst


def transpose2d(src: Tensor, nbatch: int, R: int, Cn: int, out: Optional[Tensor] = None) -> Tensor:
    dst = _out(out, (nbatch, Cn, R), src.device)
    check(_lib.load().dpot_transpose2d(src.data_ptr(), dst.data_ptr(), nbatch, R, Cn, _stream()), "transpose2d")
    return dst


def colsum(X: Tensor, M: int, N: int, ld: Optional[int] = None, out: Optional[Tensor] = None) -> Tensor:
    lib = _lib.load()
    out = _out(out, (N,), X.device)
    part = torch.empty(lib.dpot_colsum_parts(M), N, dtype=torch.float32, device=X.device)
    check(lib.dpot_colsum(X.data_ptr(), M, N, ld or N, out.data_ptr(), part.data_ptr(), _stream()), "colsum")
    return out


def group_rowsum(X: Tensor, B: int, R: int, T: int, N: int) -> Tensor:
    out = torch.empty(R, N, dtype=torch.float32, device=X.device)
    check(_lib.load().dpot_group_rowsum(X.data_ptr(), out.data_ptr(), B, R, T, N, _stream()), "group_rowsum")
    return out


def token_mean(x: Tensor) -> Tensor:
    B, T, E = x.shape
    y = torch.empty(B, E, dtype=torch.float32, device=x.device)
    check(_lib.load().dpot_token_mean(x.data_ptr(), y.data_ptr(), B, T, E, _stream()), "token_mean")
    return y


def token_mean_bwd(dy: Tensor, T: int, add: Optional[Tensor] = None) -> Tensor:
    B, E = dy.shape
    dx = torch.empty(B, T, E, dtype=torch.float32, device=dy.device)
    check(_lib.load().dpot_token_mean_bwd(dy.data_ptr(), _p(add), dx.data_ptr(), B, T, E, _stream()),
          "token_mean_bwd")
    return dx


def bias_add(x: Tensor, v: Tensor) -> Tensor:
    R, N = x.shape
    y = torch.empty_like(x)
    check(_lib.load().dpot_bias_add(x.data_ptr(), v.data_ptr(), y.data_ptr(), R, N, _stream()), "bias_add")
    return y


def tile_vec(v: Tensor, reps: int) -> Tensor:
    N = v.numel()
    y = torch.empty(reps * N, dtype=torch.float32, device=v.device)
    check(_lib.load().dpot_bias_add(None, v.data_ptr(), y.data_ptr(), reps, N, _stream()), "tile_vec")
    return y


def scale_shift(x: Tensor, scale: Tensor, shift: Tensor) -> Tensor:
    B, T, E = x.shape
    y = torch.empty_like(x)
    check(_lib.load().dpot_scale_shift(x.data_ptr(), scale.data_ptr(), shift.data_ptr(), y.data_ptr(), B, T, E,
                                       _stream()), "scale_shift")
    return y


def scale_shift_bwd(dy: Tensor, x: Tensor, scale: Tensor):
    B, T, E = x.shape
    dx = torch.empty_like(x)
    dscale = torch.empty(B, E, dtype=torch.float32, device=x.device)
    dshift = torch.empty_like(dscale)
    check(_lib.load().dpot_scale_shift_bwd(dy.data_ptr(), x.data_ptr(), scale.data_ptr(), dx.data_ptr(),
                                           dscale.data_ptr(), dshift.data_ptr(), B, T, E, _stream()), "scale_shift_bwd")
    return dx, dscale, dshift


def timeagg_scale_w(w: Tensor, gamma: Tensor, tt: Tensor) -> Tensor:
    T, E, _ = w.shape
    ws = torch.empty_like(w)
    check(_lib.load().dpot_timeagg_scale_w(w.data_ptr(), gamma.data_ptr(), tt.data_ptr(), ws.data_ptr(), T, E,
                                           _stream()), "timeagg_scale_w")
    return ws


def timeagg_scale_w_bwd(dws: Tensor, w: Tensor, gamma: Tensor, tt: Tensor, out_dw: Optional[Tensor] = None,
                        out_dgamma: Optional[Tensor] = None) -> Tuple[Tensor, Tensor]:
    T, E, _ = w.shape
    dw = _out(out_dw, (T, E, E), w.device)
    dgamma = _out(out_dgamma, (1, E), w.device)
    check(_lib.load().dpot_timeagg_scale_w_bwd(dws.data_ptr(), w.data_ptr(), gamma.data_ptr(), tt.data_ptr(),
                                               dw.data_ptr(), dgamma.data_ptr(), T, E, _stream()),
          "timeagg_scale_w_bwd")
    return dw, dgamma


def out_tail_supported(old: int, co: int, n_pixels: int) -> bool:
    return old == 32 and 0 < co <= 32 and n_pixels % 32 == 0


def out_tail_pad(w4: Tensor, b4: Tensor, co: int) -> Tuple[Tensor, Tensor]:
    return copy2d_pad(w4, co, 32, 32, 32), copy2d_pad(b4, 1, co, 1, 32).view(32)


def out_tail_fwd(upre: Tensor, w2: Tensor, b2: Tensor, w4p: Tensor, b4p: Tensor, B: int, h: int, w: int, P: int,
                 co: int, act: int) -> Tensor:
    out = torch.empty(B, h * P, w * P, co, dtype=torch.float32, device=upre.device)
    check(_lib.load().dpot_out_tail_fwd(upre.data_ptr(), w2.data_ptr(), b2.data_ptr(), w4p.data_ptr(),
                                        b4p.data_ptr(), out.data_ptr(), B, h, w, P, co, act, _stream()), "out_tail_fwd")
    return out


def colsum_scatter(X: Tensor, M: int, N: int, segments) -> None:
    lib = _lib.load()
    n = len(segments)
    starts = (C.c_int * n)(*[s for s, _ in segments])
    lens = (C.c_int * n)(*[t.numel() for _, t in segments])
    dsts = (C.c_void_p * n)(*[t.data_ptr() for _, t in segments])
    part = torch.empty(lib.dpot_colsum_parts(M) * N, dtype=torch.float32, device=X.device)
    check(lib.dpot_colsum_scatter(X.data_ptr(), M, N, N, part.data_ptr(), n, starts, lens, dsts, _stream()),
          "colsum_scatter")


def out_tail_bwd(upre: Tensor, dout: Tensor, w2: Tensor, b2: Tensor, w4p: Tensor, B: int, h: int, w: int, P: int,
                 co: int, act: int, outs=None):
    lib = _lib.load()
    rows, cols = lib.dpot_out_tail_partial_rows(B, h, w, P), lib.dpot_out_tail_partial_cols()
    dupre = torch.empty_like(upre)
    part = torch.empty(rows, cols, dtype=torch.float32, device=upre.device)
    check(lib.dpot_out_tail_bwd(upre.data_ptr(), dout.data_ptr(), w2.data_ptr(), b2.data_ptr(), w4p.data_ptr(),
                                dupre.data_ptr(), part.data_ptr(), B, h, w, P, co, act, _stream()), "out_tail_bwd")
    shapes = ((32, 32), (co, 32), (32,), (32,), (co,))
    starts = (0, 1024, 2048, 2080, 2112)
    outs = list(outs) if outs is not None else [None] * 5
    res = [_out(o, shp, upre.device) for o, shp in zip(outs, shapes)]
    colsum_scatter(part, rows, cols, list(zip(starts, res)))
    return dupre, tuple(res)


def rel_l2_fwd(x: Tensor, y: Tensor, mask: Optional[Tensor], B: int, S: int, Cc: int, Tt: int,
               stats: Optional[Tensor] = None):
    nch = _lib.load().dpot_rel_l2_chunks(S, Cc)
    if stats is None:
        stats = torch.empty(1 + nch, B, Cc, 4, dtype=torch.float32, device=x.device)
    else:
        _req(stats, "stats")
        if stats.numel() < (1 + nch) * B * Cc * 4 or stats.data_ptr() % 16:
            raise _lib.DpotHipError(f"rel_l2_fwd: the stats slot needs {(1 + nch) * B * Cc * 4} floats, 16-byte aligned")
    loss = torch.empty(1, dtype=torch.float32, device=x.device)
    check(_lib.load().dpot_rel_l2_fwd(x.data_ptr(), y.data_ptr(), _p(mask), stats.data_ptr(), loss.data_ptr(), B, S,
                                      Cc, Tt, _stream()), "rel_l2_fwd")
    return loss, stats


def rel_l2_bwd(x: Tensor, y: Tensor, mask: Optional[Tensor], stats: Tensor, gloss: Tensor, B: int, S: int, Cc: int,
               Tt: int) -> Tensor:
    dx = torch.empty_like(x)
    check(_lib.load().dpot_rel_l2_bwd(x.data_ptr(), y.data_ptr(), _p(mask), stats.data_ptr(), gloss.data_ptr(),
                                      dx.data_ptr(), B, S, Cc, Tt, _stream()), "rel_l2_bwd")
    return dx


CLS_OUT_WORDS = 4
METRICS_WORDS = 12
METRICS_FLOATS = ("l2_step", "l2_full", "cls_loss", "grad_norm")
METRICS_INTS = ("cls_correct", "cls_total", "cls_invalid", "samples", "ar_steps", "opt_steps", "nonfinite_steps")


def _req_labels(labels: Tensor, B: int) -> Tensor:
    if not labels.is_cuda:
        raise _lib.DpotHipError(f"labels must live on the MI355X (got a {labels.device} tensor): dpot_amd has no CPU path")
    if labels.dtype != torch.int64 or not labels.is_contiguous() or labels.numel() != B:
        raise _lib.DpotHipError(f"labels must be {B} contiguous int64 values, got {tuple(labels.shape)} {labels.dtype}")
    return labels


def cls_ce_fwd(logits: Tensor, labels: Tensor, out: Optional[Tensor] = None):
    _req(logits, "logits")
    if logits.dim() != 2:
        raise _lib.DpotHipError(f"logits must be [B, n_cls], got {tuple(logits.shape)}")
    B, n_cls = logits.shape
    _req_labels(labels, B)
    if out is None:
        out = torch.empty(CLS_OUT_WORDS, dtype=torch.int64, device=logits.device)
    elif out.dtype != torch.int64 or out.numel() != CLS_OUT_WORDS or not out.is_contiguous() or out.device != logits.device:
        raise _lib.DpotHipError(f"cls_ce_fwd: out must be {CLS_OUT_WORDS} contiguous int64 words on {logits.device}")
    row_stats = torch.empty(B, 2, dtype=torch.float32, device=logits.device)
    check(_lib.load().dpot_cls_ce_fwd(logits.data_ptr(), labels.data_ptr(), row_stats.data_ptr(), out.data_ptr(), B, n_cls,
                                      _stream()), "cls_ce_fwd")
    return out, row_stats


def cls_out_loss(out: Tensor) -> Tensor:
    return out.view(torch.float32)[0]


def cls_ce_bwd(logits: Tensor, labels: Tensor, row_stats: Tensor, gloss: Tensor) -> Tensor:
    _req(logits, "logits")
    _req(row_stats, "row_stats")
    _req(gloss, "gloss")
    B, n_cls = logits.shape
    _req_labels(labels, B)
    dl = torch.empty_like(logits)
    check(_lib.load().dpot_cls_ce_bwd(logits.data_ptr(), labels.data_ptr(), row_stats.data_ptr(), gloss.data_ptr(),
                                      dl.data_ptr(), B, n_cls, _stream()), "cls_ce_bwd")
    return dl


def rel_l2_stats_elems(B: int, S: int, Cc: int) -> int:
    return (1 + _lib.load().dpot_rel_l2_chunks(S, Cc)) * B * Cc * 4


class StatsTable:

    def __init__(self, stats):
        self.stats = [_req(s, "stats") for s in stats]
        if not self.stats:
            raise ValueError("StatsTable: need at least one step")
        if any(s.data_ptr() % 16 for s in self.stats):
            raise _lib.DpotHipError("StatsTable: every stats buffer must be 16-byte aligned")
        self.n_steps = len(self.stats)
        self.table = torch.tensor([s.data_ptr() for s in self.stats], dtype=torch.int64).to(self.stats[0].device)


def rel_l2_combine(stats, B: int, Cc: int, n_steps: Optional[int] = None, out: Optional[Tensor] = None) -> Tensor:
    if out is None:
        out = torch.empty(1, dtype=torch.float32, device=(stats.table if isinstance(stats, StatsTable) else stats).device)
    if isinstance(stats, StatsTable):
        n = stats.n_steps if n_steps is None else n_steps
        if not 0 < n <= stats.n_steps or any(s.numel() < B * Cc * 4 for s in stats.stats[:n]):
            raise _lib.DpotHipError("rel_l2_combine: the table does not hold n_steps buffers of >= B*C*4 floats")
        args = (stats.table.data_ptr(), None, 0)
    else:
        _req(stats, "stats")
        if stats.dim() != 2 or stats.shape[1] < B * Cc * 4:
            raise _lib.DpotHipError(f"rel_l2_combine: stats must be [n_steps, >= {B * Cc * 4}], got {tuple(stats.shape)}")
# ... 492 lines not shown
```

include/dpot_hip.h:

```cpp
#ifndef DPOT_HIP_H
#define DPOT_HIP_H

#include <stdint.h>

#ifdef __cplusplus
extern "C" {
#endif

#define DPOT_OK 0
#define DPOT_EINVAL (-1)
#define DPOT_EUNSUP (-2)
#define DPOT_EHIP (-3)

typedef void* dpot_stream_t;

enum {
  DPOT_ACT_NONE = 0,
  DPOT_ACT_GELU = 1,
  DPOT_ACT_TANH = 2,
  DPOT_ACT_SIGMOID = 3,
  DPOT_ACT_RELU = 4,
  DPOT_ACT_LEAKY_RELU = 5,
  DPOT_ACT_SOFTPLUS = 6,
  DPOT_ACT_ELU = 7,
  DPOT_ACT_SILU = 8
};

enum {
  DPOT_EPI_LINEAR = 0,
  DPOT_EPI_ACT = 1,
  DPOT_EPI_DACT = 2,
  DPOT_EPI_AFNO_WGRAD = 3
};

int dpot_version(void);
int dpot_tune(const char* key, int dflt);
const char* dpot_last_error(void);

typedef struct dpot_gemm_desc {
  const float* A;
  const float* B;
  float* C;
  int32_t M, N, K;
  int32_t batch;
  int32_t transA, transB;
  int32_t lda, ldb, ldc;
  int64_t strideA, strideB, strideC;
  const float* bias;
  int64_t strideBias;
  int32_t act;
  int32_t epi_mode;
  const float* aux;
  int32_t ldaux;
  int64_t strideAux;
  float* preact;
  int32_t ldpre;
  int64_t stridePre;
  const float* res;
  int32_t ldres;
  int32_t res_div, res_mod;
  int64_t strideRes;
  int32_t accumulate;
  int32_t splitk;
  float* workspace;
  int32_t tile;
  int32_t tag;
  float* colsum_out;
  int64_t strideColsum;
  int32_t colsum_of;
  int32_t precision;
} dpot_gemm_desc;
enum { DPOT_GEMM_F32 = 0, DPOT_GEMM_BF16X6 = 1, DPOT_GEMM_AUTO = 2, DPOT_GEMM_BF16 = 3 };

int dpot_gemm_f32(const dpot_gemm_desc* d, dpot_stream_t stream);
int64_t dpot_gemm_workspace_bytes(const dpot_gemm_desc* d);
int dpot_gemm_tn_splitk(int M, int N, int K, int batch);
int dpot_mlp_wgrad2_splitk(int T, int E, int mh);
int64_t dpot_mlp_wgrad2_ws_elems(int E, int mh, int splitk);
int dpot_mlp_wgrad2(const float* do2, const float* Hh, const float* xn2, const float* dHpre, int T, int E, int mh,
                    float* dW2, float* db2, float* dW1, float* db1, float* workspace, int splitk, dpot_stream_t stream);
int dpot_afno_wgrad2_splitk(int Mm, int nb, int bs);
int64_t dpot_afno_wgrad2_ws_elems(int nb, int bs, int splitk);
int dpot_afno_wgrad2(const float* S, const float* dO1pre, const float* O1, const float* dO2, int ld, int Mm, int nb,
                     int bs, float* dw1, float* db1, float* dw2, float* db2, float* workspace, int splitk,
                     dpot_stream_t stream);
int dpot_block_finalize(const float* afno_ws, int afno_splitk, int nb, int bs, float* dw1, float* db1, float* dw2,
                        float* db2, const float* mlp_ws, int mlp_splitk, int E, int mh, float* dW2, float* dfb2, float* dW1,
                        float* dfb1, const float* const* gn_parts, float* const* gn_dgammas, float* const* gn_dbetas,
                        int gn_jobs, int B, int Egn, const float* const* cs_parts, float* const* cs_outs, const int* cs_rows,
                        const int* cs_cols, int cs_jobs, dpot_stream_t stream);
typedef struct dpot_layout_job {
  const float* src;
  const float* add;
  float* dst;
  int32_t d0, d1, d2, v0, v1, v2;
  int64_t s0, s1, s2;
} dpot_layout_job;
int dpot_layout_jobs(const dpot_layout_job* jobs_dev, int njobs, int64_t max_elems, dpot_stream_t stream);
int dpot_gemm_auto_splitk(int M, int N, int K, int batch);
int dpot_gemm_auto_splitk2(int M, int N, int K, int batch, int precision);

int dpot_rfft2(const float* x, float* spec, int B, int h, int w, int E, int nb, int mx, int my,
               int col_weights, dpot_stream_t stream);
int dpot_irfft2(const float* spec, const float* res, float* y, int B, int h, int w, int E, int nb, int mx,
                int my, int col_weights, dpot_stream_t stream);
int dpot_rfft2_norm_supported(int h, int w, int E);
int dpot_rfft2_norm(const float* x, const float* mean, const float* rstd, const float* gamma, const float* beta, int G,
                    float* spec, int B, int h, int w, int E, int nb, int mx, int my, int col_weights,
                    dpot_stream_t stream);
int dpot_irfft2_norm(const float* spec, const float* res, const float* mean, const float* rstd, const float* gamma,
                     const float* beta, int G, float* y, int B, int h, int w, int E, int nb, int mx, int my,
                     int col_weights, dpot_stream_t stream);

int dpot_afno_pack(const float* w, const float* b, float* wbig, float* bbig, int nb, int bs,
                   dpot_stream_t stream);
int dpot_afno_pack_multi(const float* const* w, const float* const* b, float* const* wbig, float* const* bbig,
                         int njobs, int nb, int bs, dpot_stream_t stream);
int dpot_afno_unpack_grad(const float* dwbig, const float* dbbig, float* dw, float* db, int nb, int bs,
                          dpot_stream_t stream);

int64_t dpot_groupnorm_ws_elems(int B, int T, int E, int G);
int dpot_groupnorm_fwd(const float* x, const float* gamma, const float* beta, float* y, float* mean,
                       float* rstd, float* workspace, int B, int T, int E, int G, float eps, dpot_stream_t stream);
int dpot_groupnorm_bwd(const float* dy, const float* x, const float* mean, const float* rstd,
                       const float* gamma, const float* add, float* dx, float* dgamma, float* dbeta,
                       float* part , float* workspace, int B, int T, int E, int G, dpot_stream_t stream);
int dpot_groupnorm_bwd_packs_rows(int B, int T, int E, int G);
int dpot_groupnorm_bwd_packs_supported(int T, int E, int G);
int dpot_groupnorm_bwd_packs(const float* dy, const float* x, const float* mean, const float* rstd, const float* gamma,
                             const float* add, float* dx, float* part , void* dx_rows_bf16,
                             void* dx_trans_bf16, float* dx_colsum , float* workspace, int B, int T, int E,
                             int G, dpot_stream_t stream);
int dpot_groupnorm_param_grads(const float* const* parts, float* const* dgammas, float* const* dbetas, int njobs,
                               int B, int E, dpot_stream_t stream);

int dpot_gn_dft_supported(int h, int w, int E, int G);
int dpot_gn_rfft2(const float* x, const float* gamma, const float* beta, float* spec, float* mean, float* rstd, int B,
                  int h, int w, int E, int G, int nb, int mx, int my, float eps, dpot_stream_t stream);
int dpot_irfft2_gn(const float* spec, const float* x, const float* mean1, const float* rstd1, const float* gamma1,
                   const float* beta1, const float* gamma2, const float* beta2, float* y1, float* xn2, float* mean2,
                   float* rstd2, int B, int h, int w, int E, int G, int nb, int mx, int my, int col_weights, float eps,
                   dpot_stream_t stream);
int dpot_gn_bwd_rfft2(const float* dy, const float* xin, const float* mean, const float* rstd, const float* gamma,
                      float* dx, float* part, float* spec, int B, int h, int w, int E, int G, int nb, int mx, int my,
                      int col_weights, dpot_stream_t stream);
int dpot_irfft2_gn_bwd(const float* spec, const float* res, const float* xin, const float* mean, const float* rstd,
                       const float* gamma, const float* add, float* dx, float* part, int B, int h, int w, int E, int G,
                       int nb, int mx, int my, int col_weights, dpot_stream_t stream);

int dpot_afno_fused_supported(int h, int w, int E, int G, int nb, int mx, int my);
int dpot_afno_fused_fwd(const float* x, const float* gamma1, const float* beta1, const float* Wa, const float* ba,
                        const float* Wb, const float* bb, const float* gamma2, const float* beta2, float* S, float* pre,
                        float* y1, float* xn2, float* mean1, float* rstd1, float* mean2, float* rstd2, void* xn2_rows_bf16,
                        void* xn2_trans_bf16, int B, int h, int w, int E, int G, int nb, int mx, int my, int act, float eps,
                        dpot_stream_t stream);

int dpot_patchify(const float* x, const float* gx, const float* gy, const float* gt, float* A, int B, int X,
                  int Y, int T, int C, int P, dpot_stream_t stream);
int dpot_unpatchify(const float* dA, float* dx, int B, int X, int Y, int T, int C, int P,
                    dpot_stream_t stream);

int dpot_embed_supported(int C, int P, int T, int hid, int w);
int dpot_embed_wfrag_elems(void);
int dpot_embed_pack_w0(const float* w0, int hid, float* wfrag, dpot_stream_t stream);
int dpot_embed_fwd(const float* x, const float* wfrag, const float* btab, float* hpre, float* hh, int B, int X, int Y,
                   int T, int hidp, int act, dpot_stream_t stream);
int dpot_embed_wgrad_ws_elems(int B, int X, int Y);
int dpot_embed_wgrad(const float* x, const float* dhpre, float* workspace, float* dw0, int ldw, int hid, int B, int X,
                     int Y, int T, int hidp, dpot_stream_t stream);
int dpot_pixel_shuffle(const float* z, float* out, int B, int h, int w, int P, int Cc, int inverse,
                       dpot_stream_t stream);
int dpot_copy2d_pad(const float* src, int sR, int sC, float* dst, int dR, int dC, dpot_stream_t stream);
int dpot_transpose2d(const float* src, float* dst, int nbatch, int R, int C, dpot_stream_t stream);
int dpot_colsum_parts(int M);
int dpot_colsum(const float* X, int M, int N, int ld, float* out, float* part, dpot_stream_t stream);
int dpot_colsum_scatter(const float* X, int M, int N, int ld, float* part, int nseg, const int* seg_start,
                        const int* seg_len, float* const* seg_dst, dpot_stream_t stream);
int dpot_group_rowsum(const float* X, float* out, int B, int R, int T, int N, dpot_stream_t stream);
int dpot_token_mean(const float* x, float* y, int B, int T, int E, dpot_stream_t stream);
int dpot_token_mean_bwd(const float* dy, const float* add, float* dx, int B, int T, int E,
                        dpot_stream_t stream);
int dpot_small_linear_supported(int M, int N, int K);
int dpot_small_linear(const float* x, int ldx, const float* W, int ldw, const float* bias, float* y, float* pre, int ldy,
                      int M, int N, int K, int act, dpot_stream_t stream);
int dpot_bias_add(const float* x, const float* v, float* y, int R, int N, dpot_stream_t stream);
int dpot_scale_shift(const float* x, const float* scale, const float* shift, float* y, int B, int T, int E,
                     dpot_stream_t stream);
int dpot_scale_shift_bwd(const float* dy, const float* x, const float* scale, float* dx, float* dscale,
                         float* dshift, int B, int T, int E, dpot_stream_t stream);

int dpot_timeagg_scale_w(const float* w, const float* gamma, const float* tt, float* ws, int T, int E,
                         dpot_stream_t stream);
int dpot_timeagg_scale_w_bwd(const float* dws, const float* w, const float* gamma, const float* tt, float* dw,
                             float* dgamma, int T, int E, dpot_stream_t stream);

int dpot_out_tail_partial_rows(int B, int h, int w, int P);
int dpot_out_tail_partial_cols(void);
int dpot_out_tail_fwd(const float* upre, const float* w2, const float* b2, const float* w4, const float* b4,
                      float* out, int B, int h, int w, int P, int co, int act, dpot_stream_t stream);
int dpot_out_tail_bwd(const float* upre, const float* dout, const float* w2, const float* b2, const float* w4,
                      float* dupre, float* partials, int B, int h, int w, int P, int co, int act,
                      dpot_stream_t stream);

int dpot_rel_l2_chunks(int S, int C);
int dpot_rel_l2_fwd(const float* x, const float* y, const float* mask, float* stats, float* loss, int B,
                    int S, int C, int Tt, dpot_stream_t stream);
int dpot_rel_l2_bwd(const float* x, const float* y, const float* mask, const float* stats,
                    const float* gloss, float* dx, int B, int S, int C, int Tt, dpot_stream_t stream);

int dpot_sumsq(const float* g, int64_t n, float* out, float* part, int accumulate, dpot_stream_t stream);
int dpot_adam_step(float* p, const float* g, float* m, float* v, int64_t n, const float* hyper,
                   const float* sumsq, float grad_scale, dpot_stream_t stream);

int dpot_adam_stage(float* hyper, int64_t* step, float lr, double beta1, double beta2, float eps,
                    float weight_decay, float max_norm, int advance, dpot_stream_t stream);

typedef struct dpot_lamb_chunk {
  int64_t off;
  int32_t len, tensor;
} dpot_lamb_chunk;
typedef struct dpot_lamb_tensor {
  int32_t first_chunk, n_chunks;
} dpot_lamb_tensor;
int dpot_lamb_chunk_elems(void);
int dpot_lamb_step(float* p, const float* g, float* m, float* v, const float* hyper, const float* sumsq, float grad_scale,
                   const dpot_lamb_chunk* chunks_dev, int nchunks, const dpot_lamb_tensor* tensors_dev, int ntensors,
                   double* part, float* norms, int adam, dpot_stream_t stream);
int dpot_lamb_stage(float* hyper, int64_t* step, double lr, double beta1, double beta2, float eps, float weight_decay,
                    float max_norm, float clamp_value, int debias, int advance, dpot_stream_t stream);

typedef struct dpot_cls_ce_out {
  float loss;
  int32_t reserved;
  int64_t correct, valid, invalid;
} dpot_cls_ce_out;
int dpot_cls_ce_fwd(const float* logits, const int64_t* labels, float* row_stats, dpot_cls_ce_out* out, int B, int n_cls,
                    dpot_stream_t stream);
int dpot_cls_ce_bwd(const float* logits, const int64_t* labels, const float* row_stats, const float* gloss, float* dlogits,
                    int B, int n_cls, dpot_stream_t stream);
int dpot_rel_l2_combine(const float* const* stats_ptrs, const float* stats_base, int64_t step_stride, int n_steps, int B,
                        int C, float* out, dpot_stream_t stream);
typedef struct dpot_metrics {
  double l2_step, l2_full, cls_loss, grad_norm;
  int64_t cls_correct, cls_total, cls_invalid, samples, ar_steps, opt_steps, nonfinite_steps, reserved;
} dpot_metrics;
int dpot_metrics_accum(dpot_metrics* acc, const float* l2_step, const float* l2_full, const dpot_cls_ce_out* cls,
                       int n_cls_out, const float* sumsq, float grad_scale, int64_t samples, int64_t ar_steps,
                       int64_t opt_steps, dpot_stream_t stream);

int dpot_noise_chunks(int S, int C);
int dpot_noise_inject(const float* xx, const float* eps, float* out, float* norms, float noise_scale, int B,
                      int S, int C, dpot_stream_t stream);
int dpot_noise_inject_rng(const float* xx, float* out, float* norms, uint64_t* rng_state, float noise_scale, int B,
                          int S, int C, dpot_stream_t stream);

int dpot_afno_mlp2_supported(int nb, int bs);
int dpot_afno_mlp3_supported(int nb, int bs);
int dpot_afno_mlp2(const float* X, const float* Wa, const float* ba, const float* Wb, const float* bb,
                   const float* aux, float* pre, float* mid, float* Y, int M, int nb, int bs, int ldx, int ldo,
                   int act, int mode, int layout, dpot_stream_t stream);
int dpot_afno_mlp6_supported(int nb, int bs);
int64_t dpot_afno_pack6_elems(int nb, int bs);
int dpot_afno_pack6(const float* wbig, void* fwd6, void* bwd6, int nitems, int nb, int bs, dpot_stream_t stream);
int dpot_afno_mlp6(const float* X, const void* Wa6, const float* ba, const void* Wb6, const float* bb, const float* aux,
                   float* pre, float* mid, float* Y, int M, int nb, int bs, int ldx, int ldo, int act, int mode,
                   dpot_stream_t stream);
int dpot_afno_block_weights(const float* wbig, float* fwd, float* bwd, int nmat, int N, dpot_stream_t stream);

typedef struct dpot_afno_pack_job {
  const float* w;
  const float* b;
  float* wbig;
  float* bbig;
  float* fwd;
  float* bwd;
} dpot_afno_pack_job;
int dpot_afno_pack_all(const dpot_afno_pack_job* jobs_dev, int njobs, int nb, int bs, int layout, dpot_stream_t stream);

int dpot_noise_inject_bwd(const float* xx, const float* eps, const uint64_t* rng_state, const float* g,
                          const float* norms, float* dx, float* part, float noise_scale, int B, int S, int C,
                          dpot_stream_t stream);

int dpot_window_slide(const float* xx, const float* im, float* out, int64_t rows, int T, int Tb, int C,
                      dpot_stream_t stream);
int dpot_window_slide_bwd(const float* dout, float* dxx, float* dim, int64_t rows, int T, int Tb, int C,
                          dpot_stream_t stream);

typedef struct dpot_pack_job {
  const float* src;
  float* dst;
  int32_t rows, K, ld, trans;
} dpot_pack_job;
int dpot_panel_pack_weights(const dpot_pack_job* jobs_dev, int njobs, int max_elems, dpot_stream_t stream);
int dpot_gemm_panel_supported(int M, int N, int K);
int dpot_gemm_panel(const float* A, int lda, const float* Wpacked, const float* bias, const float* aux, int ldaux,
                    const float* res, int ldres, float* pre, int ldpre, float* C, int ldc, int M, int N, int K,
                    int act, int epi_mode, dpot_stream_t stream);

int64_t dpot_bf16_packed_elems(int rows, int K, int planes);
int dpot_bf16_pack_rows(const float* src, int ld, int rows, int K, int trans, int planes, void* dst,
                        dpot_stream_t stream);
int dpot_bf16_pack_both_supported(int rows, int K);
int dpot_bf16_pack_both(const float* src, int ld, int rows, int K, void* dst_rows, void* dst_trans, float* colsum_part,
                        dpot_stream_t stream);
int dpot_bf16_pack_both_norm(const float* src, int ld, int rows, int K, const float* mean, const float* rstd,
                             const float* gamma, const float* beta, int rows_per_sample, int G, void* dst_rows,
                             void* dst_trans, dpot_stream_t stream);
int dpot_bf16_pack_jobs(const dpot_pack_job* jobs_dev, int njobs, int max_elems, int planes, dpot_stream_t stream);
typedef struct dpot_adam_pack_job {
  int64_t off;
  void* dst_rows;
  void* dst_trans;
  int32_t R, K, tile0, pad_;
} dpot_adam_pack_job;
typedef struct dpot_adam_range {
  int64_t start, len;
} dpot_adam_range;
int dpot_adam_pack_supported(int rows, int K);
int dpot_adam_step_packs(float* p, const float* g, float* m, float* v, const float* hyper, const float* sumsq,
                         float grad_scale, const dpot_adam_pack_job* jobs_dev, const int32_t* tile_job_dev, int ntiles,
                         const dpot_adam_range* ranges_dev, int nranges, int max_range_len, dpot_stream_t stream);
int dpot_gemm_bf16p_supported(int M, int N, int K);
int dpot_gemm_bf16p_kernel_kind(int M, int N, int K, int splitk, int planes, int packed_outputs);
int dpot_gemm_bf16p(const void* Apacked, const void* Wpacked, const float* bias, const float* aux, int ldaux,
                    const float* res, int ldres, float* pre, int ldpre, float* C, int ldc, int M, int N, int K, int act,
                    int epi_mode, int planes, int splitk, float* workspace, void* out_rows, void* out_trans,
                    float* colsum_part, void* dact_out, const void* dact_in, dpot_stream_t stream);
int dpot_gemm_bf16p_pair_wanted(int M0, int N0, int M1, int N1, int K);
int dpot_gemm_bf16p_pair_splitk(int M0, int N0, int M1, int N1, int K);
int dpot_gemm_bf16p_pair(const void* A0, const void* W0, float* C0, int ldc0, int M0, int N0, const void* A1,
                         const void* W1, float* C1, int ldc1, int M1, int N1, int K, int splitk, float* workspace,
                         dpot_stream_t stream);
int dpot_gemm_bf16p_splitk(int M, int N, int K);

typedef struct dpot_sample_desc {
  const float* data;
  int32_t H, W, T, C;
  int32_t t0;
  int32_t reserved;
} dpot_sample_desc;
int dpot_resize_pad_window(const dpot_sample_desc* samples_dev, int nsamples, float* xx, float* yy, int res, int t_in,
                           int t_ar, int n_channels, int down_h, int down_w, dpot_stream_t stream);

int dpot_spectral_resize_pad(int n, int output_rows);
int dpot_spectral_resize(const float* in, float* out, const float* axT, const float* ayT, const float* byT, const float* u,
// ... 16 lines not shown
```

Baseline: 10540.

## Group independent embed-stage GEMMs and reductions into single grouped launches

Adds a grouped GEMM kernel that runs up to eight independent small GEMM or split-K sum jobs in one launch, with each workgroup picking its job from a prefix table. It also adds a grouped reduction launch and a fused time-aggregation scale plus weight-sum kernel. The embed stage's weight-only products and gradients are batched per dependency level to cut launch count and small-kernel underutilisation. In exchange the grouped kernel uses a generic 64x64 tile with runtime branching, which may be slower than the specialised per-shape kernels.

```diff
diff --git a/dpot_amd/_lib.py b/dpot_amd/_lib.py
--- a/dpot_amd/_lib.py
+++ b/dpot_amd/_lib.py
@@ -65,6 +65,29 @@
                 ("s2", C.c_int64)]
 
 
+class GemmJob(C.Structure):
+    _fields_ = [
+        ("kind", C.c_int32),
+        ("A", c_fp), ("B", c_fp), ("C", c_fp),
+        ("M", C.c_int32), ("N", C.c_int32), ("K", C.c_int32),
+        ("batch", C.c_int32),
+        ("transA", C.c_int32), ("transB", C.c_int32),
+        ("lda", C.c_int32), ("ldb", C.c_int32), ("ldc", C.c_int32),
+        ("strideA", c_i64), ("strideB", c_i64), ("strideC", c_i64),
+        ("bias", c_fp), ("strideBias", c_i64),
+        ("act", C.c_int32), ("epi_mode", C.c_int32),
+        ("res", c_fp), ("ldres", C.c_int32), ("res_mod", C.c_int32), ("strideRes", c_i64),
+        ("trans_out", C.c_int32), ("nstore", C.c_int32),
+        ("colsum_part", c_fp),
+        ("kranges", C.c_int32),
+    ]
+
+
+class SumJob(C.Structure):
+    _fields_ = [("X", c_fp), ("out", c_fp), ("kind", C.c_int32), ("B", C.c_int32), ("R", C.c_int32), ("T", C.c_int32),
+                ("N", C.c_int32)]
+
+
 class AfnoPackJob(C.Structure):
     _fields_ = [("w", c_fp), ("b", c_fp), ("wbig", c_fp), ("bbig", c_fp), ("fwd", c_fp), ("bwd", c_fp)]
 
@@ -80,6 +103,10 @@
     "dpot_last_error": (C.c_char_p, []),
     "dpot_gemm_f32": (c_i, [C.POINTER(GemmDesc), c_fp]),
     "dpot_gemm_workspace_bytes": (c_i64, [C.POINTER(GemmDesc)]),
+    "dpot_gemm_group": (c_i, [C.POINTER(GemmJob), c_i, c_fp]),
+    "dpot_gemm_group_wgs": (c_i64, [C.POINTER(GemmJob)]),
+    "dpot_sum_group": (c_i, [C.POINTER(SumJob), c_i, c_fp]),
+    "dpot_timeagg_scale_w_sum": (c_i, [c_fp] * 5 + [c_i, c_i, c_fp]),
     "dpot_gemm_auto_splitk": (c_i, [c_i, c_i, c_i, c_i]),
     "dpot_gemm_auto_splitk2": (c_i, [c_i, c_i, c_i, c_i, c_i]),
     "dpot_rfft2": (c_i, [c_fp, c_fp] + [c_i] * 8 + [c_fp]),
diff --git a/dpot_amd/build.py b/dpot_amd/build.py
--- a/dpot_amd/build.py
+++ b/dpot_amd/build.py
@@ -10,7 +10,7 @@
 CSRC = os.path.join(HERE, "csrc")
 LIBDIR = os.path.join(HERE, "lib")
 LIB = os.path.join(LIBDIR, "libdpot_hip.so")
-SOURCES = ["core.hip", "gemm.hip", "gemm_panel.hip", "gemm_tn.hip", "gemm_bf16p.hip", "afno_mlp.hip", "afno_mlp6.hip", "afno_fused.hip", "dft.hip", "norm.hip", "gn_dft.hip", "misc.hip", "loss_opt.hip", "metrics.hip", "tail.hip", "data.hip", "embed.hip", "resize.hip", "evalmetrics.hip"]
+SOURCES = ["core.hip", "gemm.hip", "gemm_group.hip", "gemm_panel.hip", "gemm_tn.hip", "gemm_bf16p.hip", "afno_mlp.hip", "afno_mlp6.hip", "afno_fused.hip", "dft.hip", "norm.hip", "gn_dft.hip", "misc.hip", "loss_opt.hip", "metrics.hip", "tail.hip", "data.hip", "embed.hip", "resize.hip", "evalmetrics.hip"]
 FLAGS = ["--offload-arch=gfx950", "-O3", "-std=c++17", "-fPIC", "-Wall", "-Wno-unused-function",
          "-Wno-pass-failed"]
 EXTRA_FLAGS = {"afno_mlp6.hip": ["-fno-slp-vectorize"]}
@@ -33,7 +33,7 @@
 def build(force: bool = False, verbose: bool = True) -> str:
     hipcc = _hipcc()
     os.makedirs(LIBDIR, exist_ok=True)
-    hdrs = [os.path.join(CSRC, "common.h"), os.path.join(CSRC, "dft_fast.h"), os.path.join(CSRC, "gemm_split.h"), os.path.join(CSRC, "gemm_epi.h"), os.path.join(CSRC, "gemm_bf16p_common.h"), os.path.join(os.path.dirname(HERE), "include", "dpot_hip.h")]
+    hdrs = [os.path.join(CSRC, "common.h"), os.path.join(CSRC, "dft_fast.h"), os.path.join(CSRC, "gemm_split.h"), os.path.join(CSRC, "gemm_epi.h"), os.path.join(CSRC, "gemm_tile.h"), os.path.join(CSRC, "gemm_bf16p_common.h"), os.path.join(os.path.dirname(HERE), "include", "dpot_hip.h")]
     objs, jobs = [], []
     for src in SOURCES:
         s = os.path.join(CSRC, src)
diff --git a/dpot_amd/csrc/gemm.hip b/dpot_amd/csrc/gemm.hip
--- a/dpot_amd/csrc/gemm.hip
+++ b/dpot_amd/csrc/gemm.hip
@@ -1,93 +1,8 @@
 #include "common.h"
 #include "gemm_epi.h"
+#include "gemm_tile.h"
 
 namespace dpot {
-
-constexpr int BK = 32;
-constexpr int KPAD = 4;
-
-template <int R, bool VEC>
-__device__ __forceinline__ void load_kcontig(float4 (&reg)[R / 32], const float* __restrict__ base, int ld,
-                                             int r0, int rmax, int k0, int kmax, int tid) {
-#pragma unroll
-  for (int i = 0; i < R / 32; ++i) {
-    const int f = tid + 256 * i;
-    const int r = r0 + (f >> 3);
-    const int k = k0 + ((f & 7) << 2);
-    const float* row = base + (long long)min(r, rmax - 1) * ld;
-    float4 v;
-    if constexpr (VEC) {
-      v = *reinterpret_cast<const float4*>(row + min(k, kmax - 4));
-    } else {
-      const int kl = kmax - 1;
-      v.x = row[min(k + 0, kl)]; v.y = row[min(k + 1, kl)]; v.z = row[min(k + 2, kl)]; v.w = row[min(k + 3, kl)];
-    }
-    reg[i] = v;
-  }
-}
-template <int R, bool VEC>
-__device__ __forceinline__ void load_rcontig(float4 (&reg)[R / 32], const float* __restrict__ base, int ld,
-                                             int r0, int rmax, int k0, int kmax, int tid) {
-  constexpr int F4_PER_ROW = R / 4;
-#pragma unroll
-  for (int i = 0; i < R / 32; ++i) {
-    const int f = tid + 256 * i;
-    const int k = k0 + f / F4_PER_ROW;
-    const int r = r0 + ((f % F4_PER_ROW) << 2);
-    const float* row = base + (long long)min(k, kmax - 1) * ld;
-    float4 v;
-    if constexpr (VEC) {
-      v = *reinterpret_cast<const float4*>(row + min(r, rmax - 4));
-    } else {
-      const int rl = rmax - 1;
-      v.x = row[min(r + 0, rl)]; v.y = row[min(r + 1, rl)]; v.z = row[min(r + 2, rl)]; v.w = row[min(r + 3, rl)];
-    }
-    reg[i] = v;
-  }
-}
-template <int R>
-__device__ __forceinline__ void zero_tail_kcontig(float* lds, int krem, int tid) {
-  for (int idx = tid; idx < R * BK; idx += 256) {
-    const int r = idx / BK, k = idx % BK;
-    if (k >= krem) lds[r * (BK + KPAD) + k] = 0.f;
-  }
-}
-template <int R>
-__device__ __forceinline__ void zero_tail_rcontig(float* lds, int krem, int tid) {
-  for (int idx = tid + krem * R; idx < BK * R; idx += 256) lds[idx] = 0.f;
-}
-template <int R>
-__device__ __forceinline__ void store_kcontig(float* lds, const float4 (&reg)[R / 32], int tid) {
-#pragma unroll
-  for (int i = 0; i < R / 32; ++i) {
-    const int f = tid + 256 * i;
-    *reinterpret_cast<float4*>(&lds[(f >> 3) * (BK + KPAD) + ((f & 7) << 2)]) = reg[i];
-  }
-}
-template <int R>
-__device__ __forceinline__ void store_rcontig(float* lds, const float4 (&reg)[R / 32], int tid) {
-  constexpr int F4_PER_ROW = R / 4;
-#pragma unroll
-  for (int i = 0; i < R / 32; ++i) {
-    const int f = tid + 256 * i;
-    *reinterpret_cast<float4*>(&lds[(f / F4_PER_ROW) * R + ((f % F4_PER_ROW) << 2)]) = reg[i];
-  }
-}
-
-template <int R, bool KCONTIG>
-struct TileLds {
-  static constexpr int floats = KCONTIG ? R * (BK + KPAD) : BK * R;
-};
-
-template <int R, bool KCONTIG>
-__device__ __forceinline__ float4 frag(const float* lds, int row, int kk, int kh) {
-  if constexpr (KCONTIG) {
-    return *reinterpret_cast<const float4*>(&lds[row * (BK + KPAD) + kk + 4 * kh]);
-  } else {
-    const float* p = &lds[(kk + 4 * kh) * R + row];
-    return make_float4(p[0], p[R], p[2 * R], p[3 * R]);
-  }
-}
 
 template <int BM, int BN, bool TA, bool TB, bool VEC, int TAG>
 __global__ __launch_bounds__(256) void gemm_f32_kernel(const GemmArgs p) {
diff --git a/dpot_amd/csrc/gemm_group.hip b/dpot_amd/csrc/gemm_group.hip
--- /dev/null
+++ b/dpot_amd/csrc/gemm_group.hip
@@ -0,0 +1,275 @@
+#include "common.h"
+#include "gemm_epi.h"
+#include "gemm_tile.h"
+
+namespace dpot {
+
+constexpr int GT = 64;
+constexpr int STAGE_LD = 33;
+constexpr int SUM_ELEMS_PER_WG = 1024;
+
+struct GroupJob {
+  const float* A;
+  const float* B;
+  float* C;
+  const float* bias;
+  const float* res;
+  float* cs_part;
+  long long sA, sB, sC, sBias, sRes;
+  int M, N, K, batch;
+  int lda, ldb, ldc, ldres, res_mod;
+  int kind, ta, tb, vec;
+  int act, mode;
+  int trans_out, nstore;
+  int kranges, kper;
+  int tilesM, tilesN;
+};
+
+struct GroupArgs {
+  int njobs;
+  int first[DPOT_GROUP_MAX_JOBS + 1];
+  GroupJob jobs[DPOT_GROUP_MAX_JOBS];
+};
+
+__device__ __forceinline__ float job_epi(const GroupJob& j, int b, int m, int n, float v) {
+  if (j.bias) v += j.bias[b * j.sBias + n];
+  if (j.mode == DPOT_EPI_ACT) v = act_fwd(j.act, v);
+  if (j.res) v += j.res[b * j.sRes + (long long)(j.res_mod > 0 ? m % j.res_mod : m) * j.ldres + n];
+  return v;
+}
+__device__ __forceinline__ void job_store(const GroupJob& j, int b, int m, int n, float v) {
+  if (n >= j.nstore) return;
+  float* c = j.C + b * j.sC;
+  if (j.trans_out) c[(long long)n * j.ldc + m] = v; else c[(long long)m * j.ldc + n] = v;
+}
+
+template <bool TA, bool TB, bool VEC>
+__device__ __forceinline__ void tile_mainloop(f32x16& acc, const float* __restrict__ A, const float* __restrict__ B, int lda,
+                                              int ldb, int M, int N, int m0, int n0, int kbeg, int kend, float* As,
+                                              float* Bs, int tid) {
+  constexpr bool A_KC = !TA;
+  constexpr bool B_KC = TB;
+  const int lane = tid & 63, wave = tid >> 6;
+  const int wm = wave >> 1, wn = wave & 1;
+  const int li = lane & 31, kh = lane >> 5;
+  const int nk = (kend > kbeg) ? (kend - kbeg + BK - 1) / BK : 0;
+  float4 ra[GT / 32], rb[GT / 32];
+  auto gload = [&](int k0) {
+    if constexpr (A_KC) load_kcontig<GT, VEC>(ra, A, lda, m0, M, k0, kend, tid);
+    else load_rcontig<GT, VEC>(ra, A, lda, m0, M, k0, kend, tid);
+    if constexpr (B_KC) load_kcontig<GT, VEC>(rb, B, ldb, n0, N, k0, kend, tid);
+    else load_rcontig<GT, VEC>(rb, B, ldb, n0, N, k0, kend, tid);
+  };
+  auto sstore = [&](int k0) {
+    if constexpr (A_KC) store_kcontig<GT>(As, ra, tid); else store_rcontig<GT>(As, ra, tid);
+    if constexpr (B_KC) store_kcontig<GT>(Bs, rb, tid); else store_rcontig<GT>(Bs, rb, tid);
+    if (k0 + BK > kend) {
+      __syncthreads();
+      const int krem = kend - k0;
+      if constexpr (A_KC) zero_tail_kcontig<GT>(As, krem, tid); else zero_tail_rcontig<GT>(As, krem, tid);
+      if constexpr (B_KC) zero_tail_kcontig<GT>(Bs, krem, tid); else zero_tail_rcontig<GT>(Bs, krem, tid);
+    }
+  };
+  if (nk == 0) return;
+  gload(kbeg);
+  sstore(kbeg);
+  __syncthreads();
+  for (int kt = 0; kt < nk; ++kt) {
+    if (kt + 1 < nk) gload(kbeg + (kt + 1) * BK);
+#pragma unroll
+    for (int kk = 0; kk < BK; kk += 8) {
+      const float4 af = frag<GT, A_KC>(As, wm * 32 + li, kk, kh);
+      const float4 bf = frag<GT, B_KC>(Bs, wn * 32 + li, kk, kh);
+      acc = __builtin_amdgcn_mfma_f32_32x32x2f32(af.x, bf.x, acc, 0, 0, 0);
+      acc = __builtin_amdgcn_mfma_f32_32x32x2f32(af.y, bf.y, acc, 0, 0, 0);
+      acc = __builtin_amdgcn_mfma_f32_32x32x2f32(af.z, bf.z, acc, 0, 0, 0);
+      acc = __builtin_amdgcn_mfma_f32_32x32x2f32(af.w, bf.w, acc, 0, 0, 0);
+    }
+    __syncthreads();
+    if (kt + 1 < nk) {
+      sstore(kbeg + (kt + 1) * BK);
+      __syncthreads();
+    }
+  }
+}
+
+__device__ __forceinline__ void sum_job(const GroupJob& j, int wg, int tid) {
+  const long long MN = (long long)j.M * j.N;
+  const long long total = MN * j.batch;
+  const long long base = (long long)wg * SUM_ELEMS_PER_WG;
+  for (int i = tid; i < SUM_ELEMS_PER_WG; i += 256) {
+    const long long idx = base + i;
+    if (idx >= total) break;
+    float v = 0.f;
+    for (int p = 0; p < j.kranges; ++p) v += j.A[p * j.sA + idx];
+    const int b = (int)(idx / MN);
+    const long long rem = idx - (long long)b * MN;
+    const int m = (int)(rem / j.N), n = (int)(rem % j.N);
+    job_store(j, b, m, n, job_epi(j, b, m, n, v));
+  }
+}
+
+__global__ __launch_bounds__(256) void gemm_group_kernel(const GroupArgs p) {
+  constexpr int OPER_FLOATS = 2 * GT * (BK + KPAD);
+  static_assert(OPER_FLOATS >= 4 * 32 * STAGE_LD, "the staging slabs reuse the operand slabs");
+  __shared__ __attribute__((aligned(16))) float smem[OPER_FLOATS + 256];
+  const int tid = threadIdx.x;
+  int ji = 0;
+  for (int q = 1; q < p.njobs; ++q)
+    if ((int)blockIdx.x >= p.first[q]) ji = q;
+  const GroupJob& j = p.jobs[ji];
+  const int wg = blockIdx.x - p.first[ji];
+  if (j.kind == 1) {
+    sum_job(j, wg, tid);
+    return;
+  }
+  const int lane = tid & 63, wave = tid >> 6;
+  const int wm = wave >> 1, wn = wave & 1;
+  const int li = lane & 31, kh = lane >> 5;
+  const int ntiles = j.tilesM * j.tilesN;
+  const int tile = wg % ntiles;
+  const int zb = (wg / ntiles) % j.batch, kr = wg / (ntiles * j.batch);
+  const int tm_idx = tile / j.tilesN, tn_idx = tile % j.tilesN;
+  const int m0 = tm_idx * GT, n0 = tn_idx * GT;
+  const float* A = j.A + zb * j.sA;
+  const float* B = j.B + zb * j.sB;
+  const int kbeg = kr * j.kper;
+  int kend = kbeg + j.kper;
+  if (kend > j.K) kend = j.K;
+  float* As = smem;
+  float* Bs = smem + (j.ta ? BK * GT : GT * (BK + KPAD));
+
+  f32x16 acc;
+#pragma unroll
+  for (int r = 0; r < 16; ++r) acc[r] = 0.f;
+  const int key = (j.ta ? 2 : 0) | (j.tb ? 1 : 0);
+#define DPOT_GROUP_LOOP(TA_, TB_)                                                                                      \
+  do {                                                                                                                 \
+    if (j.vec) tile_mainloop<TA_, TB_, true>(acc, A, B, j.lda, j.ldb, j.M, j.N, m0, n0, kbeg, kend, As, Bs, tid);      \
+    else tile_mainloop<TA_, TB_, false>(acc, A, B, j.lda, j.ldb, j.M, j.N, m0, n0, kbeg, kend, As, Bs, tid);           \
+  } while (0)
+  switch (key) {
+    case 0: DPOT_GROUP_LOOP(false, false); break;
+    case 1: DPOT_GROUP_LOOP(false, true); break;
+    case 2: DPOT_GROUP_LOOP(true, false); break;
+    default: DPOT_GROUP_LOOP(true, true); break;
+  }
+#undef DPOT_GROUP_LOOP
+
+  __syncthreads();
+  const int m0f = m0 + wm * 32, n0f = n0 + wn * 32;
+  float* stage = smem + wave * (32 * STAGE_LD);
+  float* cs = smem + OPER_FLOATS;
+  const int n = n0f + li;
+  float csum = 0.f;
+  if (j.kranges > 1) {
+    float* ws = j.C + ((long long)kr * j.batch + zb) * j.M * j.N;
+#pragma unroll
+    for (int r = 0; r < 16; ++r) {
+      const int m = m0f + 4 * kh + (r & 3) + 8 * (r >> 2);
+      if (m < j.M && n < j.N) ws[(long long)m * j.N + n] = acc[r];
+    }
+    return;
+  }
+#pragma unroll
+  for (int r = 0; r < 16; ++r) {
+    const int row = 4 * kh + (r & 3) + 8 * (r >> 2);
+    const int m = m0f + row;
+    float v = acc[r];
+    if (m < j.M && n < j.N) {
+      v = job_epi(j, zb, m, n, v);
+      if (n < j.nstore) csum += v;
+    }
+    stage[row * STAGE_LD + li] = v;
+  }
+  __builtin_amdgcn_fence(__ATOMIC_RELEASE, "wavefront");
+  __builtin_amdgcn_wave_barrier();
+  __builtin_amdgcn_fence(__ATOMIC_ACQUIRE, "wavefront");
+  if (j.trans_out) {
+    const int m = m0f + li;
+    for (int it = 0; it < 16; ++it) {
+      const int col = 2 * it + kh;
+      if (m < j.M && n0f + col < j.N) job_store(j, zb, m, n0f + col, stage[li * STAGE_LD + col]);
+    }
+  } else {
+    for (int it = 0; it < 16; ++it) {
+      const int row = 2 * it + kh;
+      if (m0f + row < j.M && n < j.N) job_store(j, zb, m0f + row, n, stage[row * STAGE_LD + li]);
+    }
+  }
+  if (j.cs_part) {
+    cs[(wave * 2 + kh) * 32 + li] = csum;
+    __syncthreads();
+    if (tid < GT) {
+      const int w = tid >> 5, c = tid & 31;
+      const float s = (cs[((0 * 2 + w) * 2 + 0) * 32 + c] + cs[((0 * 2 + w) * 2 + 1) * 32 + c]) +
+                      (cs[((1 * 2 + w) * 2 + 0) * 32 + c] + cs[((1 * 2 + w) * 2 + 1) * 32 + c]);
+      if (n0 + tid < j.nstore) j.cs_part[(long long)tm_idx * j.N + n0 + tid] = s;
+    }
+  }
+}
+
+}
+
+using namespace dpot;
+
+extern "C" int64_t dpot_gemm_group_wgs(const dpot_gemm_job* d) {
+  if (!d || d->M <= 0 || d->N <= 0 || d->batch <= 0) return 0;
+  if (d->kind == DPOT_JOB_SUM) return cdiv64((int64_t)d->M * d->N * d->batch, SUM_ELEMS_PER_WG);
+  const int kr = d->kranges > 1 ? d->kranges : 1;
+  return (int64_t)cdiv(d->M, GT) * cdiv(d->N, GT) * d->batch * kr;
+}
+
+extern "C" int dpot_gemm_group(const dpot_gemm_job* jobs, int njobs, dpot_stream_t stream) {
+  DPOT_REQUIRE(jobs != nullptr && njobs > 0 && njobs <= DPOT_GROUP_MAX_JOBS, "gemm_group: 1..%d jobs, got %d",
+               DPOT_GROUP_MAX_JOBS, njobs);
+  GroupArgs p;
+  memset(&p, 0, sizeof(p));
+  p.njobs = njobs;
+  long long total = 0;
+  for (int i = 0; i < njobs; ++i) {
+    const dpot_gemm_job* d = &jobs[i];
+    GroupJob& g = p.jobs[i];
+    DPOT_REQUIRE(d->kind == DPOT_JOB_GEMM || d->kind == DPOT_JOB_SUM, "gemm_group: job %d: bad kind %d", i, d->kind);
+    DPOT_REQUIRE(d->A && d->C && d->M > 0 && d->N > 0 && d->batch > 0, "gemm_group: job %d: bad shape or null operand", i);
+    DPOT_REQUIRE(d->epi_mode == DPOT_EPI_LINEAR || d->epi_mode == DPOT_EPI_ACT, "gemm_group: job %d: epilogue mode %d", i,
+                 d->epi_mode);
+    DPOT_REQUIRE(d->nstore >= 0 && d->nstore <= d->N, "gemm_group: job %d: nstore=%d outside [0, N]", i, d->nstore);
+    const int nstore = d->nstore > 0 ? d->nstore : d->N;
+    DPOT_REQUIRE(d->ldc >= (d->trans_out ? d->M : nstore), "gemm_group: job %d: ldc=%d too small", i, d->ldc);
+    DPOT_REQUIRE(!d->res || d->ldres >= d->N, "gemm_group: job %d: ldres=%d too small", i, d->ldres);
+    g.A = d->A; g.B = d->B; g.C = d->C;
+    g.bias = d->bias; g.res = d->res; g.cs_part = d->colsum_part;
+    g.sA = d->strideA; g.sB = d->strideB; g.sC = d->strideC; g.sBias = d->strideBias; g.sRes = d->strideRes;
+    g.M = d->M; g.N = d->N; g.K = d->K; g.batch = d->batch;
+    g.lda = d->lda; g.ldb = d->ldb; g.ldc = d->ldc; g.ldres = d->ldres; g.res_mod = d->res_mod;
+    g.kind = d->kind; g.ta = d->transA != 0; g.tb = d->transB != 0;
+    g.act = d->act; g.mode = d->epi_mode;
+    g.trans_out = d->trans_out != 0; g.nstore = nstore;
+    g.tilesM = cdiv(d->M, GT); g.tilesN = cdiv(d->N, GT);
+    if (d->kind == DPOT_JOB_SUM) {
+      DPOT_REQUIRE(d->kranges >= 1 && !d->colsum_part, "gemm_group: job %d: a sum job needs kranges = parts >= 1", i);
+      g.kranges = d->kranges;
+    } else {
+      DPOT_REQUIRE(d->B && d->K > 0, "gemm_group: job %d: bad K or null B", i);
+      DPOT_REQUIRE(d->lda >= (d->transA ? d->M : d->K), "gemm_group: job %d: lda=%d too small", i, d->lda);
+      DPOT_REQUIRE(d->ldb >= (d->transB ? d->K : d->N), "gemm_group: job %d: ldb=%d too small", i, d->ldb);
+      g.kranges = d->kranges > 1 ? d->kranges : 1;
+      DPOT_REQUIRE(g.kranges == 1 || (!d->bias && !d->res && !d->colsum_part && !d->trans_out && d->nstore == 0 &&
+                                      d->epi_mode == DPOT_EPI_LINEAR),
+                   "gemm_group: job %d: a K-ranged job writes raw partials; its epilogue belongs to the sum job", i);
+      DPOT_REQUIRE(!d->colsum_part || d->batch == 1, "gemm_group: job %d: column sums need batch = 1", i);
+      g.kper = cdiv(cdiv(d->K, BK), g.kranges) * BK;
+      const int contA = d->transA ? d->M : d->K, contB = d->transB ? d->K : d->N;
+      const bool vecA = aligned16(d->A) && d->lda % 4 == 0 && contA % 4 == 0 && d->strideA % 4 == 0;
+      const bool vecB = aligned16(d->B) && d->ldb % 4 == 0 && contB % 4 == 0 && d->strideB % 4 == 0;
+      g.vec = vecA && vecB;
+    }
+    p.first[i] = (int)total;
+    total += dpot_gemm_group_wgs(d);
+    DPOT_REQUIRE(total < (1ll << 30), "gemm_group: grid too large");
+  }
+  for (int i = njobs; i <= DPOT_GROUP_MAX_JOBS; ++i) p.first[i] = (int)total;
+  hipLaunchKernelGGL(gemm_group_kernel, dim3((unsigned)total), dim3(256), 0, as_stream(stream), p);
+  return check_launch("gemm_group_kernel");
+}
diff --git a/dpot_amd/csrc/gemm_tile.h b/dpot_amd/csrc/gemm_tile.h
--- /dev/null
+++ b/dpot_amd/csrc/gemm_tile.h
@@ -0,0 +1,92 @@
+#pragma once
+#include "common.h"
+
+namespace dpot {
+
+constexpr int BK = 32;
+constexpr int KPAD = 4;
+
+template <int R, bool VEC>
+__device__ __forceinline__ void load_kcontig(float4 (&reg)[R / 32], const float* __restrict__ base, int ld,
+                                             int r0, int rmax, int k0, int kmax, int tid) {
+#pragma unroll
+  for (int i = 0; i < R / 32; ++i) {
+    const int f = tid + 256 * i;
+    const int r = r0 + (f >> 3);
+    const int k = k0 + ((f & 7) << 2);
+    const float* row = base + (long long)min(r, rmax - 1) * ld;
+    float4 v;
+    if constexpr (VEC) {
+      v = *reinterpret_cast<const float4*>(row + min(k, kmax - 4));
+    } else {
+      const int kl = kmax - 1;
+      v.x = row[min(k + 0, kl)]; v.y = row[min(k + 1, kl)]; v.z = row[min(k + 2, kl)]; v.w = row[min(k + 3, kl)];
+    }
+    reg[i] = v;
+  }
+}
+template <int R, bool VEC>
+__device__ __forceinline__ void load_rcontig(float4 (&reg)[R / 32], const float* __restrict__ base, int ld,
+                                             int r0, int rmax, int k0, int kmax, int tid) {
+  constexpr int F4_PER_ROW = R / 4;
+#pragma unroll
+  for (int i = 0; i < R / 32; ++i) {
+    const int f = tid + 256 * i;
+    const int k = k0 + f / F4_PER_ROW;
+    const int r = r0 + ((f % F4_PER_ROW) << 2);
+    const float* row = base + (long long)min(k, kmax - 1) * ld;
+    float4 v;
+    if constexpr (VEC) {
+      v = *reinterpret_cast<const float4*>(row + min(r, rmax - 4));
+    } else {
+      const int rl = rmax - 1;
+      v.x = row[min(r + 0, rl)]; v.y = row[min(r + 1, rl)]; v.z = row[min(r + 2, rl)]; v.w = row[min(r + 3, rl)];
+    }
+    reg[i] = v;
+  }
+}
+template <int R>
+__device__ __forceinline__ void zero_tail_kcontig(float* lds, int krem, int tid) {
+  for (int idx = tid; idx < R * BK; idx += 256) {
+    const int r = idx / BK, k = idx % BK;
+    if (k >= krem) lds[r * (BK + KPAD) + k] = 0.f;
+  }
+}
+template <int R>
+__device__ __forceinline__ void zero_tail_rcontig(float* lds, int krem, int tid) {
+  for (int idx = tid + krem * R; idx < BK * R; idx += 256) lds[idx] = 0.f;
+}
+template <int R>
+__device__ __forceinline__ void store_kcontig(float* lds, const float4 (&reg)[R / 32], int tid) {
+#pragma unroll
+  for (int i = 0; i < R / 32; ++i) {
+    const int f = tid + 256 * i;
+    *reinterpret_cast<float4*>(&lds[(f >> 3) * (BK + KPAD) + ((f & 7) << 2)]) = reg[i];
+  }
+}
+template <int R>
+__device__ __forceinline__ void store_rcontig(float* lds, const float4 (&reg)[R / 32], int tid) {
+  constexpr int F4_PER_ROW = R / 4;
+#pragma unroll
+  for (int i = 0; i < R / 32; ++i) {
+    const int f = tid + 256 * i;
+    *reinterpret_cast<float4*>(&lds[(f / F4_PER_ROW) * R + ((f % F4_PER_ROW) << 2)]) = reg[i];
+  }
+}
+
+template <int R, bool KCONTIG>
+struct TileLds {
+  static constexpr int floats = KCONTIG ? R * (BK + KPAD) : BK * R;
+};
+
+template <int R, bool KCONTIG>
+__device__ __forceinline__ float4 frag(const float* lds, int row, int kk, int kh) {
+  if constexpr (KCONTIG) {
+    return *reinterpret_cast<const float4*>(&lds[row * (BK + KPAD) + kk + 4 * kh]);
+  } else {
+    const float* p = &lds[(kk + 4 * kh) * R + row];
+    return make_float4(p[0], p[R], p[2 * R], p[3 * R]);
+  }
+}
+
+}
diff --git a/dpot_amd/csrc/misc.hip b/dpot_amd/csrc/misc.hip
--- a/dpot_amd/csrc/misc.hip
+++ b/dpot_amd/csrc/misc.hip
@@ -227,6 +227,69 @@
   const long long off = ((long long)t * E + i) * E;
   for (int j = threadIdx.x; j < E; j += 256) ws[off + j] = w[off + j] * cs;
 }
+__global__ __launch_bounds__(256) void timeagg_scale_w_sum_kernel(const float* __restrict__ w, const float* __restrict__ gamma,
+                                                                  const float* __restrict__ tt, float* __restrict__ ws,
+                                                                  float* __restrict__ wsum, int T, int E) {
+  const int i = blockIdx.x;
+  const float ga = gamma[i];
+  for (int j = threadIdx.x; j < E; j += 256) {
+    float s = 0.f;
+    for (int t = 0; t < T; ++t) {
+      const long long off = ((long long)t * E + i) * E + j;
+      const float v = w[off] * cosf(tt[t] * ga);
+      ws[off] = v;
+      s += v;
+    }
+    wsum[(long long)i * E + j] = s;
+  }
+}
+
+struct SumArgs {
+  int njobs;
+  int first[DPOT_SUM_MAX_JOBS + 1];
+  dpot_sum_job jobs[DPOT_SUM_MAX_JOBS];
+};
+__global__ __launch_bounds__(256) void sum_group_kernel(const SumArgs p) {
+  __shared__ float red[4][64];
+  int ji = 0;
+  for (int q = 1; q < p.njobs; ++q)
+    if ((int)blockIdx.x >= p.first[q]) ji = q;
+  const dpot_sum_job& j = p.jobs[ji];
+  const int wg = blockIdx.x - p.first[ji];
+  const int tc = threadIdx.x & 63, tr = threadIdx.x >> 6;
+  const int N = j.N;
+  const float* __restrict__ X = j.X;
+  if (j.kind == 0) {
+    const int nbx = (N + 63) / 64;
+    const int n = (wg % nbx) * 64 + tc, r = wg / nbx;
+    const int B = j.B, R = j.R, T = j.T;
+    float s0 = 0.f, s1 = 0.f;
+    if (n < N) {
+      const int BT = B * T;
+      int q = tr;
+      for (; q + 4 < BT; q += 8) {
+        const int b0 = q / T, t0 = q % T, b1 = (q + 4) / T, t1 = (q + 4) % T;
+        s0 += X[(((long long)b0 * R + r) * T + t0) * N + n];
+        s1 += X[(((long long)b1 * R + r) * T + t1) * N + n];
+      }
+      for (; q < BT; q += 4) s0 += X[(((long long)(q / T) * R + r) * T + (q % T)) * N + n];
+    }
+    red[tr][tc] = s0 + s1;
+    __syncthreads();
+    if (tr == 0 && n < N) j.out[(long long)r * N + n] = (red[0][tc] + red[1][tc]) + (red[2][tc] + red[3][tc]);
+  } else {
+    const int chunk = (j.R + j.B - 1) / j.B;
+    const int rbeg = wg * chunk;
+    const int rend = rbeg + chunk < j.R ? rbeg + chunk : j.R;
+    float s = 0.f;
+    if (tc < N)
+      for (int r = rbeg + tr; r < rend; r += 4) s += X[(long long)r * j.T + tc];
+    red[tr][tc] = s;
+    __syncthreads();
+    if (tr == 0 && tc < N) j.out[(long long)wg * N + tc] = (red[0][tc] + red[1][tc]) + (red[2][tc] + red[3][tc]);
+  }
+}
+
 __global__ __launch_bounds__(256) void timeagg_scale_w_bwd_kernel(const float* __restrict__ dws, const float* __restrict__ w,
                                                                   const float* __restrict__ gamma,
                                                                   const float* __restrict__ tt, float* __restrict__ dw,
@@ -537,6 +600,35 @@
   return check_launch("timeagg_scale_w_kernel");
 }
 
+extern "C" int dpot_timeagg_scale_w_sum(const float* w, const float* gamma, const float* tt, float* ws, float* wsum, int T,
+                                        int E, dpot_stream_t stream) {
+  DPOT_REQUIRE(w && gamma && tt && ws && wsum && T > 0 && E > 0, "timeagg_scale_w_sum: bad argument");
+  hipLaunchKernelGGL(timeagg_scale_w_sum_kernel, dim3(E), dim3(256), 0, as_stream(stream), w, gamma, tt, ws, wsum, T, E);
+  return check_launch("timeagg_scale_w_sum_kernel");
+}
+
+extern "C" int dpot_sum_group(const dpot_sum_job* jobs, int njobs, dpot_stream_t stream) {
+  DPOT_REQUIRE(jobs != nullptr && njobs > 0 && njobs <= DPOT_SUM_MAX_JOBS, "sum_group: 1..%d jobs, got %d",
+               DPOT_SUM_MAX_JOBS, njobs);
+  SumArgs p;
+  memset(&p, 0, sizeof(p));
+  p.njobs = njobs;
+  long long total = 0;
+  for (int i = 0; i < njobs; ++i) {
+    const dpot_sum_job& d = jobs[i];
+    DPOT_REQUIRE(d.X && d.out && d.B > 0 && d.R > 0 && d.T > 0 && d.N > 0 && (d.kind == 0 || d.kind == 1),
+                 "sum_group: job %d: bad argument", i);
+    DPOT_REQUIRE(d.kind == 0 || (d.N <= 64 && d.T >= d.N), "sum_group: job %d: column-sum partials need N <= 64 <= ld", i);
+    p.jobs[i] = d;
+    p.first[i] = (int)total;
+    total += d.kind == 0 ? (long long)cdiv(d.N, 64) * d.R : d.B;
+    DPOT_REQUIRE(total < (1ll << 30), "sum_group: grid too large");
+  }
+  for (int i = njobs; i <= DPOT_SUM_MAX_JOBS; ++i) p.first[i] = (int)total;
+  hipLaunchKernelGGL(sum_group_kernel, dim3((unsigned)total), dim3(256), 0, as_stream(stream), p);
+  return check_launch("sum_group_kernel");
+}
+
 extern "C" int dpot_timeagg_scale_w_bwd(const float* dws, const float* w, const float* gamma, const float* tt,
                                         float* dw, float* dgamma, int T, int E, dpot_stream_t stream) {
   DPOT_REQUIRE(dws && w && gamma && tt && dw && T > 0 && E > 0, "timeagg_scale_w_bwd: bad argument");
diff --git a/dpot_amd/functional.py b/dpot_amd/functional.py
--- a/dpot_amd/functional.py
+++ b/dpot_amd/functional.py
@@ -100,18 +100,32 @@
         w2p = ops.copy2d_pad(w2, E, hid, E, hidp)
         posT = ops.transpose2d(pos, 1, E, tok).view(tok, E)
         posb = ops.bias_add(posT, b2)
-    ws = ops.timeagg_scale_w(taw, tagamma, tt) if tagamma is not None else taw
+    grouped = ops.embed_group_enabled()
     V = torch.empty(T * hidp, E, dtype=torch.float32, device=dev)
-    ops.gemm(w2p, ws, V, hidp, E, E, transA=True, lda=hidp, ldb=E, ldc=E, batch=T, strideA=0, strideB=E * E,
-             strideC=hidp * E)
-    wsum = ops.colsum(ws, T, E * E).view(E, E)
     cc = torch.empty(tok, E, dtype=torch.float32, device=dev)
-    ops.gemm(posb, wsum, cc, tok, E, E, lda=E, ldb=E, ldc=E)
     wfrag = bt = None
     if grid is not None:
         kg = grid.shape[1]
         wfrag = ops.embed_pack_w0(w0)
         bt = torch.empty(grid.shape[0], hidp, dtype=torch.float32, device=dev)
+    kw_V = dict(transA=True, lda=hidp, ldb=E, ldc=E, batch=T, strideA=0, strideB=E * E, strideC=hidp * E)
+    kw_c = dict(lda=E, ldb=E, ldc=E)
+    if grouped:
+        if tagamma is not None:
+            ws, wsum = ops.timeagg_scale_w_sum(taw, tagamma, tt)
+        else:
+            ws, wsum = taw, ops.colsum(taw, T, E * E).view(E, E)
+        jobs = [ops.gemm_job(w2p, ws, V, hidp, E, E, **kw_V), ops.gemm_job(posb, wsum, cc, tok, E, E, **kw_c)]
+        if grid is not None:
+            jobs.append(ops.gemm_job(grid, w0p[:, K0 - kg:], bt, grid.shape[0], hidp, kg, transB=True, lda=kg, ldb=K0,
+                                     ldc=hidp, bias=b0p))
+        ops.gemm_group(jobs)
+        return w0p, b0p, w2p, posb, ws, V, wsum, cc, wfrag, bt, grid
+    ws = ops.timeagg_scale_w(taw, tagamma, tt) if tagamma is not None else taw
+    ops.gemm(w2p, ws, V, hidp, E, E, **kw_V)
+    wsum = ops.colsum(ws, T, E * E).view(E, E)
+    ops.gemm(posb, wsum, cc, tok, E, E, **kw_c)
+    if grid is not None:
         ops.gemm(grid, w0p[:, K0 - kg:], bt, grid.shape[0], hidp, kg, transB=True, lda=kg, ldb=K0, ldc=hidp, bias=b0p)
     return w0p, b0p, w2p, posb, ws, V, wsum, cc, wfrag, bt, grid
 
@@ -151,22 +165,13 @@
         return Yl.view(B, tok, E)
 
     @staticmethod
-    @ops.with_ctx_precision
-    def backward(ctx, dY):
-        _check_epoch(ctx, "EmbedFn")
+    def _backward_single(ctx, dY, dHpre, dV):
         A0, Hpre, Hh, w0p, w2p, ws, V, wsum, posb, taw, tagamma, tt, grid = ctx.saved_tensors
         B, X, Y, T, Cc, P, h, w, hid, hidp, E, K0, act = ctx.dims
         s_pos, s_w0, s_b0, s_w2, s_b2, s_taw, s_gamma = ctx.sinks
         tok = h * w
         M, M0 = B * tok, B * tok * T
         dev = dY.device
-        dY = dY.contiguous().view(M, E)
-        dHpre = torch.empty(M0, hidp, dtype=torch.float32, device=dev)
-        ops.gemm(dY, V, dHpre, M, T * hidp, E, transB=True, lda=E, ldb=E, ldc=T * hidp, act=act, mode=EPI_DACT,
-                 aux=Hpre, ldaux=T * hidp)
-        dV = torch.empty(T * hidp, E, dtype=torch.float32, device=dev)
-        ops.gemm(Hh, dY, dV, T * hidp, E, M, transA=True, lda=T * hidp, ldb=E, ldc=E,
-                 splitk=ops.auto_splitk(T * hidp, E, M, tn=True))
         dc = ops.group_rowsum(dY, B, tok, 1, E)
         dwsum = torch.empty(E, E, dtype=torch.float32, device=dev)
         ops.gemm(posb, dc, dwsum, E, E, tok, transA=True, lda=E, ldb=E, ldc=E, splitk=ops.auto_splitk(E, E, tok, tn=True))
@@ -205,6 +210,100 @@
             dw0p = ops.linear_bwd_weight(dHpre, A0)
         if not ctx.implicit:
             dw0 = s_w0.done(ops.copy2d_pad(dw0p, hidp, K0, hid, K0, out=s_w0.out()).view(hid, Cc + 3, P, P))
+        return dpos, dw0, db0, dw2, db2, dtaw, dgamma
+
+    @staticmethod
+    def _backward_grouped(ctx, dY, dHpre, dV):
+        A0, Hpre, Hh, w0p, w2p, ws, V, wsum, posb, taw, tagamma, tt, grid = ctx.saved_tensors
+        B, X, Y, T, Cc, P, h, w, hid, hidp, E, K0, act = ctx.dims
+        s_pos, s_w0, s_b0, s_w2, s_b2, s_taw, s_gamma = ctx.sinks
+        tok = h * w
+        M, M0 = B * tok, B * tok * T
+        dev = dY.device
+        new = lambda *shape: torch.empty(*shape, dtype=torch.float32, device=dev)
+        implicit = ctx.implicit
+        dc = new(tok, E)
+        sums = [(dY, dc, 0, B, tok, 1, E)]
+        if implicit:
+            nparts = min(256, (M0 + 63) // 64)
+            dHs, db0_part = new(tok * T, hidp), new(nparts, hid)
+            sums += [(dHpre, dHs, 0, B, tok * T, 1, hidp), (dHpre, db0_part, 1, nparts, M0, hidp, hid)]
+        ops.sum_group(sums)
+        dwsum, dw2_t = new(E, E), new(T, E, hidp)
+        dposT = ops._out(s_pos.out(), (E, tok), dev)
+        tiles_tok = (tok + 63) // 64
+        db2_part = new(tiles_tok, E)
+        jobs = [ops.gemm_job(posb, dc, dwsum, E, E, tok, transA=True, lda=E, ldb=E, ldc=E),
+                ops.gemm_job(dc, wsum, dposT, tok, E, E, transB=True, lda=E, ldb=E, ldc=tok, trans_out=True,
+                             colsum_part=db2_part),
+                ops.gemm_job(ws, dV, dw2_t, E, hidp, E, transB=True, lda=E, ldb=E, ldc=hidp, batch=T, strideA=E * E,
+                             strideB=hidp * E, strideC=E * hidp)]
+        if implicit:
+            kg = grid.shape[1]
+            dw0 = ops._out(s_w0.out(), (hid, K0), dev)
+            db0 = ops._out(s_b0.out(), (hid,), dev)
+            kr = max(1, min(16, (tok * T + 31) // 32 // 8))
+            kw_g = dict(transA=True, lda=hidp, ldb=kg)
+            if kr > 1:
+                dw0g_part = new(kr, hid, kg)
+                jobs.append(ops.gemm_job(dHs, grid, dw0g_part, hid, kg, tok * T, ldc=kg, kranges=kr, **kw_g))
+            else:
+                jobs.append(ops.gemm_job(dHs, grid, dw0[:, K0 - kg:], hid, kg, tok * T, ldc=K0, **kw_g))
+            jobs.append(ops.sum_job(db0_part, db0, 1, hid, nparts, stride=hid, ldc=hid))
+        ops.gemm_group(jobs)
+        dws = ops._out(s_taw.out() if tagamma is None else None, (T, E, E), dev)
+        dw2 = ops._out(s_w2.out(), (E, hid), dev)
+        db2 = ops._out(s_b2.out(), (E,), dev)
+        jobs = [ops.gemm_job(w2p, dV, dws, E, E, hidp, lda=hidp, ldb=E, ldc=E, batch=T, strideA=0, strideB=hidp * E,
+                             strideC=E * E, res=dwsum, ldres=E, strideRes=0),
+                ops.sum_job(dw2_t, dw2, E, hidp, T, stride=E * hidp, ldc=hid, nstore=hid),
+                ops.sum_job(db2_part, db2, 1, E, tiles_tok, stride=E, ldc=E)]
+        if implicit and kr > 1:
+            jobs.append(ops.sum_job(dw0g_part, dw0[:, K0 - kg:], hid, kg, kr, stride=hid * kg, ldc=K0))
+        ops.gemm_group(jobs)
+        dpos = s_pos.done(dposT.view(1, E, h, w))
+        db2 = s_b2.done(db2)
+        dw2 = s_w2.done(dw2.view(E, hid, 1, 1))
+        if tagamma is not None:
+            dtaw, dgamma = ops.timeagg_scale_w_bwd(dws, taw, tagamma, tt, out_dw=s_taw.out(), out_dgamma=s_gamma.out())
+            dtaw, dgamma = s_taw.done(dtaw), s_gamma.done(dgamma)
+        else:
+            dtaw, dgamma = s_taw.done(dws), None
+        if implicit:
+            db0 = s_b0.done(db0)
+            ops.embed_wgrad(A0, dHpre, dw0, hid)
+            dw0 = s_w0.done(dw0.view(hid, Cc + 3, P, P))
+        elif hid == hidp:
+            dw0p, db0 = ops.linear_bwd_wb(dHpre, A0, None, s_b0.out())
+            db0 = s_b0.done(db0)
+        else:
+            db0 = s_b0.done(ops.colsum(dHpre, M0, hid, ld=hidp, out=s_b0.out()))
+            dw0p = ops.linear_bwd_weight(dHpre, A0)
+        if not implicit:
+            dw0 = s_w0.done(ops.copy2d_pad(dw0p, hidp, K0, hid, K0, out=s_w0.out()).view(hid, Cc + 3, P, P))
+        return dpos, dw0, db0, dw2, db2, dtaw, dgamma
+
+    @staticmethod
+    @ops.with_ctx_precision
+    def backward(ctx, dY):
+        _check_epoch(ctx, "EmbedFn")
+        A0, Hpre, Hh, w0p, w2p, ws, V, wsum, posb, taw, tagamma, tt, grid = ctx.saved_tensors
+        B, X, Y, T, Cc, P, h, w, hid, hidp, E, K0, act = ctx.dims
+        s_pos, s_w0, s_b0, s_w2, s_b2, s_taw, s_gamma = ctx.sinks
+        tok = h * w
+        M, M0 = B * tok, B * tok * T
+        dev = dY.device
+        dY = dY.contiguous().view(M, E)
+        dHpre = torch.empty(M0, hidp, dtype=torch.float32, device=dev)
+        ops.gemm(dY, V, dHpre, M, T * hidp, E, transB=True, lda=E, ldb=E, ldc=T * hidp, act=act, mode=EPI_DACT,
+                 aux=Hpre, ldaux=T * hidp)
+        dV = torch.empty(T * hidp, E, dtype=torch.float32, device=dev)
+        ops.gemm(Hh, dY, dV, T * hidp, E, M, transA=True, lda=T * hidp, ldb=E, ldc=E,
+                 splitk=ops.auto_splitk(T * hidp, E, M, tn=True))
+        if ops.embed_group_enabled():
+            dpos, dw0, db0, dw2, db2, dtaw, dgamma = EmbedFn._backward_grouped(ctx, dY, dHpre, dV)
+        else:
+            dpos, dw0, db0, dw2, db2, dtaw, dgamma = EmbedFn._backward_single(ctx, dY, dHpre, dV)
         dx = None
         if ctx.needs_input_grad[0]:
             dA0 = ops.linear_bwd_data(dHpre, w0p)
diff --git a/dpot_amd/ops.py b/dpot_amd/ops.py
--- a/dpot_amd/ops.py
+++ b/dpot_amd/ops.py
@@ -129,7 +129,9 @@
     "packs": (1, "0 = bf16 packs by separate pack passes only: none from the one-launch AFNO layer, the GroupNorm backward or Adam"),
     "pack_both": (1, "0 = bf16 channel MLP without the pack-both path (one pack pass per operand form, fp32 pre-activation saved)"),
     "fused_small": (1, "0 = separate small launches: per-block reduce launches, eight layout launches, torch ops for the cls head"),
-    "embed_implicit": (1, "0 = explicit patch matrix + GEMM instead of the implicit-GEMM patch embedding"),
+    "embed_implicit": (1, "0 = explicit patch matrix + GEMM instead of the implicit-GEMM patch embedding; 2 = as 1, but the embed "
+                          "stage's weight-only products and their gradients on a launch (or split-K launch pair) each, as under 0, "
+                          "instead of the grouped launches per dependency level (gemm_group / sum_group)"),
     "mixer6": (1, "bf16x6 mixer kernel afno_mlp6 under gemm_precision 'auto' / 'bf16x6': 1 = where it measured faster (96 channels "
                   "per block: DPOT-L), 2 = wherever supported (also 128), 0 = never (the fp32 matrix-core kernels)"),
 }
@@ -229,6 +231,44 @@
     return C_
 
 
+JOB_GEMM, JOB_SUM = 0, 1
+GROUP_MAX_JOBS = 8
+
+
+def gemm_job(A: Tensor, B: Tensor, C_: Tensor, M: int, N: int, K: int, *, transA: bool = False, transB: bool = False,
+             lda: int, ldb: int, ldc: int, batch: int = 1, strideA: int = 0, strideB: int = 0, strideC: int = 0,
+             bias: Optional[Tensor] = None, strideBias: int = 0, act: int = 0, mode: int = EPI_LINEAR,
+             res: Optional[Tensor] = None, ldres: int = 0, res_mod: int = 0, strideRes: int = 0, trans_out: bool = False,
+             nstore: int = 0, colsum_part: Optional[Tensor] = None, kranges: int = 1):
+    return _lib.GemmJob(JOB_GEMM, A.data_ptr(), B.data_ptr(), C_.data_ptr(), M, N, K, batch, int(transA), int(transB), lda,
+                        ldb, ldc, strideA, strideB, strideC, _p(bias), strideBias, act, mode, _p(res), ldres, res_mod,
+                        strideRes, int(trans_out), nstore, _p(colsum_part), kranges)
+
+
+def sum_job(parts_: Tensor, C_: Tensor, M: int, N: int, parts: int, *, stride: int, ldc: int, batch: int = 1,
+            strideC: int = 0, bias: Optional[Tensor] = None, strideBias: int = 0, act: int = 0, mode: int = EPI_LINEAR,
+            res: Optional[Tensor] = None, ldres: int = 0, res_mod: int = 0, strideRes: int = 0, trans_out: bool = False,
+            nstore: int = 0):
+    return _lib.GemmJob(JOB_SUM, parts_.data_ptr(), None, C_.data_ptr(), M, N, 0, batch, 0, 0, 0, 0, ldc, stride, 0, strideC,
+                        _p(bias), strideBias, act, mode, _p(res), ldres, res_mod, strideRes, int(trans_out), nstore, None,
+                        parts)
+
+
+def embed_group_enabled() -> bool:
+    return tune("embed_implicit") == 1 and _cur_gemm() in (GEMM_F32, GEMM_AUTO)
+
+
+def gemm_group(jobs) -> None:
+    arr = (_lib.GemmJob * len(jobs))(*jobs)
+    check(_lib.load().dpot_gemm_group(arr, len(jobs), _stream()), "gemm_group")
+
+
+def sum_group(jobs) -> None:
+    arr = (_lib.SumJob * len(jobs))(*(_lib.SumJob(X.data_ptr(), out.data_ptr(), kind, B, R, T, N)
+                                      for X, out, kind, B, R, T, N in jobs))
+    check(_lib.load().dpot_sum_group(arr, len(jobs), _stream()), "sum_group")
+
+
 def panel_enabled() -> bool:
     return tune("panel") != 0 and _cur_gemm() == GEMM_F32
 
@@ -1032,6 +1072,15 @@
     check(_lib.load().dpot_timeagg_scale_w(w.data_ptr(), gamma.data_ptr(), tt.data_ptr(), ws.data_ptr(), T, E,
                                            _stream()), "timeagg_scale_w")
     return ws
+
+
+def timeagg_scale_w_sum(w: Tensor, gamma: Tensor, tt: Tensor) -> Tuple[Tensor, Tensor]:
+    T, E, _ = w.shape
+    ws = torch.empty_like(w)
+    wsum = torch.empty(E, E, dtype=torch.float32, device=w.device)
+    check(_lib.load().dpot_timeagg_scale_w_sum(w.data_ptr(), gamma.data_ptr(), tt.data_ptr(), ws.data_ptr(), wsum.data_ptr(),
+                                               T, E, _stream()), "timeagg_scale_w_sum")
+    return ws, wsum
 
 
 def timeagg_scale_w_bwd(dws: Tensor, w: Tensor, gamma: Tensor, tt: Tensor, out_dw: Optional[Tensor] = None,
diff --git a/include/dpot_hip.h b/include/dpot_hip.h
--- a/include/dpot_hip.h
+++ b/include/dpot_hip.h
@@ -97,6 +97,40 @@
   int64_t s0, s1, s2;
 } dpot_layout_job;
 int dpot_layout_jobs(const dpot_layout_job* jobs_dev, int njobs, int64_t max_elems, dpot_stream_t stream);
+enum { DPOT_JOB_GEMM = 0, DPOT_JOB_SUM = 1 };
+#define DPOT_GROUP_MAX_JOBS 8
+typedef struct dpot_gemm_job {
+  int32_t kind;
+  const float* A;
+  const float* B;
+  float* C;
+  int32_t M, N, K;
+  int32_t batch;
+  int32_t transA, transB;
+  int32_t lda, ldb, ldc;
+  int64_t strideA, strideB, strideC;
+  const float* bias;
+  int64_t strideBias;
+  int32_t act;
+  int32_t epi_mode;
+  const float* res;
+  int32_t ldres;
+  int32_t res_mod;
+  int64_t strideRes;
+  int32_t trans_out;
+  int32_t nstore;
+  float* colsum_part;
+  int32_t kranges;
+} dpot_gemm_job;
+int dpot_gemm_group(const dpot_gemm_job* jobs_host, int njobs, dpot_stream_t stream);
+int64_t dpot_gemm_group_wgs(const dpot_gemm_job* job);
+#define DPOT_SUM_MAX_JOBS 4
+typedef struct dpot_sum_job {
+  const float* X;
+  float* out;
+  int32_t kind, B, R, T, N;
+} dpot_sum_job;
+int dpot_sum_group(const dpot_sum_job* jobs_host, int njobs, dpot_stream_t stream);
 int dpot_gemm_auto_splitk(int M, int N, int K, int batch);
 int dpot_gemm_auto_splitk2(int M, int N, int K, int batch, int precision);
 
@@ -191,6 +225,8 @@
 
 int dpot_timeagg_scale_w(const float* w, const float* gamma, const float* tt, float* ws, int T, int E,
                          dpot_stream_t stream);
+int dpot_timeagg_scale_w_sum(const float* w, const float* gamma, const float* tt, float* ws, float* wsum, int T, int E,
+                             dpot_stream_t stream);
 int dpot_timeagg_scale_w_bwd(const float* dws, const float* w, const float* gamma, const float* tt, float* dw,
                              float* dgamma, int T, int E, dpot_stream_t stream);
 
```

Measured after the change: 10560 (median of 6 runs). Within noise of the previous version (+0.2%).
